# IML-DKFZ/values

Measured on AMD Instinct MI355X. Metric: uncertainty-volumes/sec (64^3, T=10 MC-dropout), higher is better.
Workload: dtype f32; 1 GPU; C2: 64^3 1-channel volumes, UNet3D(initial_filter_size=8, 2 classes), T=10 MC-dropout passes + fused softmax/entropy/MI/variance/argmax reduction; dropout=hash bit generator, new seed every step, weights=torch default init, seed 123

## Files before the change

include/values_amd.h:

```cpp
#ifndef VALUES_AMD_H
#define VALUES_AMD_H

#include <stddef.h>
#include <stdint.h>

#ifdef __cplusplus
extern "C" {
#endif

typedef void* vx_stream_t;

enum {
  VX_OK = 0,
  VX_E_NULL = -1,
  VX_E_SHAPE = -2,
  VX_E_DTYPE = -3,
  VX_E_WORKSPACE = -4,
  VX_E_ALIGN = -5
};

enum { VX_F32 = 0, VX_F64 = 1 };
enum { VX_ACT_NONE = 0, VX_ACT_LRELU = 1 , VX_ACT_RELU = 2 };
enum { VX_DROP_NONE = 0, VX_DROP_HASH = 1, VX_DROP_MASK = 2 };

// ... 107 lines not shown
  const float* acc_in;
  int32_t acc_pitch;
  int32_t out_planar, in_planar;
  int32_t products;
} vx_conv3d_args;
int64_t vx_conv3d_upfused_packed_floats(void);
int vx_pack_conv3d_upfused(const float* w1_torch, const float* b1, const float* up_w_torch, const float* up_b, float* packed,
                           vx_stream_t stream);
int vx_conv3d_k3_prologue_ok(int D, int H, int W, int Cin, int Cout);
int vx_conv3d_k3_upfuse_ok(int D, int H, int W, int Cin, int Cout);
int64_t vx_convT_zc16_packed_floats(void);
int64_t vx_conv3d_upfused_zc16_packed_floats(void);
int vx_pack_conv3d_upfused_zc16(const float* w1_torch, const float* up_w_torch, const float* up_b, float* packed, vx_stream_t stream);
int vx_pack_convT_zc16(const float* w_torch , float* packed, vx_stream_t stream);
int vx_conv3d_k3_skip_prologue_ok(int D, int H, int W, int Cin, int Cout, int xblk);
int vx_conv3d_k3_acc_ok(int D, int H, int W, int Cin, int Cout);
int vx_conv3d_k3_planar_ok(int D, int H, int W, int Cin, int Cout);
int vx_conv3d_k3_poolfuse_ok(int D, int H, int W, int Cin, int Cout);
int vx_conv3d_k3_presplit_ok(int D, int H, int W, int Cin, int Cout);
int vx_conv3d_k3_poolfin_ok(int Cin, int Cout);
int vx_prenorm_split(float* x, const float* mean, const float* rstd, int N, int64_t nvox, float scale, vx_stream_t stream);
int vx_pool_finish(const float* pool_raw, const uint32_t* pool_flags, const float* mean, const float* rstd, float* out,
                   int out_pitch, int N, int64_t voxels_per_sample, int drop_scale2, vx_stream_t stream);
int vx_pool_finish_z(const float* pool_raw, const uint32_t* pool_flags, const float* mean, const float* rstd, float* out,
                     int out_pitch, int N, int Dp, int64_t plane_voxels, int drop_scale2, vx_stream_t stream);
int vx_conv3d_k3_pool_layout(int D, int H, int W, int Cin, int Cout);
int vx_conv3d_k3_tiles(int D, int H, int W);
int vx_conv3d_k3_tiles_for(int D, int H, int W, int Cout);
int vx_conv3d_k3(const vx_conv3d_args* a, vx_stream_t stream);
int vx_conv3d_k3_head_fusable(int Cin, int Cout);
int vx_conv3d_k3_route(const vx_conv3d_args* a, char* kernel_name, int cap);

int vx_conv3d_k3_c1_tiles(int D, int H, int W);
int vx_conv3d_k3_c1(const float* in, const float* w_torch , const float* bias, float* out,
                    int out_pitch, int N, int D, int H, int W, int Cout, int repeat, const int32_t* src,
                    const int32_t* flip, float* stats_partial, vx_stream_t stream);

int vx_pack_input_cl8(const float* in, float* out, int N, int Cin, int D, int H, int W, int repeat, const int32_t* src,
                      const int32_t* flip, vx_stream_t stream);

int vx_instnorm_finalize(const float* stats_partial, int N, int ntiles, int C, int64_t nvox, float eps,
                         float* mean, float* rstd, vx_stream_t stream);

typedef struct vx_norm_args {
  const float* x; int32_t x_pitch;
  const float* mean; const float* rstd;
  float* out; int32_t out_pitch, out_coff;
  float* pool_out; int32_t pool_pitch;
  int32_t N, D, H, W, C;
  int32_t act, drop_mode; uint32_t drop_seed, drop_layer; const uint8_t* drop_mask;
  int32_t out_xblk, out_half;
  int32_t x_xblk, x_half;
  const uint32_t* seed_dev;
  uint32_t* range_flag;
} vx_norm_args;
int vx_norm_act_drop_pool(const vx_norm_args* a, vx_stream_t stream);
typedef struct vx_stat_src {
  const float* stats_partial; int32_t tiles; float eps; int64_t count;
  float* mean_out; float* rstd_out;
} vx_stat_src;
int vx_norm_act_drop_pool_stats(const vx_norm_args* a, const vx_stat_src* st, vx_stream_t stream);
int vx_prenorm_split_stats(float* x, const vx_stat_src* st, int N, int64_t nvox, float scale, vx_stream_t stream);
int vx_zero(void* p, int64_t bytes, vx_stream_t stream);
int vx_pool_finish_z_stats(const float* pool_raw, const uint32_t* pool_flags, const vx_stat_src* st, float* out, int out_pitch,
                           int N, int Dp, int64_t plane_voxels, int drop_scale2, vx_stream_t stream);
int vx_norm_act_drop_pool_bcast(const vx_norm_args* a, int x_repeat, vx_stream_t stream);
typedef struct vx_norm_route_info {
  int32_t grid_x, grid_y;
  uint32_t per_sample;
  uint32_t magic_pw, magic_c4, magic_rh;
} vx_norm_route_info;
int vx_norm_act_drop_pool_route(const vx_norm_args* a, int x_repeat, const vx_stat_src* st, char* kernel_name, int cap,
                                vx_norm_route_info* info);

typedef struct vx_convT_args {
  const float* in; int32_t in_pitch;
  const float* w_packed; const float* bias;
  float* out; int32_t out_pitch, out_coff;
  int32_t N, D, H, W, Cin, Cout;
  int32_t act, drop_mode; uint32_t drop_seed, drop_layer; const uint8_t* drop_mask;
  int32_t out_xblk, out_half;
  uint32_t* range_flag;
  const uint32_t* seed_dev;
} vx_convT_args;
int vx_convT_k2s2(const vx_convT_args* a, vx_stream_t stream);
typedef struct vx_convT_route_info {
  int32_t grid_x, grid_y;
} vx_convT_route_info;
int vx_convT_k2s2_route(const vx_convT_args* a, char* kernel_name, int cap, vx_convT_route_info* info);

int vx_conv1x1_ncdhw(const float* in, int in_pitch, const float* w, const float* bias, float* out, int N, int D,
                     int H, int W, int F, int C, const int32_t* dst, const int32_t* flip, vx_stream_t stream);

typedef struct vx_unet3d_weights {
  const float* conv_w[18];
  const float* conv_b[18];
  const float* up_w[4];
  const float* up_b[4];
  const float* final_w;
  const float* final_b;
  int32_t F;
  int32_t num_classes;
  int32_t conv_family[18];
  int32_t in_channels;
  int32_t no_instancenorm;
  const float* up_fused;
  const float* split_w[2];
  int32_t split_family;
  const float* up3_zc16;
  const float* up3_fused;
} vx_unet3d_weights;

typedef struct vx_unet3d_run {
  const float* x;
  int32_t N, D, H, W;
  int32_t repeat;
  const int32_t* src;
  const int32_t* flip;
  const int32_t* dst;
  int32_t drop_mode;
  uint32_t seed;
  const uint8_t* masks[17];
  float* logits;
  void* workspace; size_t workspace_bytes;
  uint32_t* range_flag;
  const uint32_t* seed_dev;
} vx_unet3d_run;

size_t vx_unet3d_workspace_bytes(int N, int D, int H, int W, int F);
int vx_unet3d_forward(const vx_unet3d_weights* w, const vx_unet3d_run* r, vx_stream_t stream);
int vx_unet3d_forward_profiled(const vx_unet3d_weights* w, const vx_unet3d_run* r, vx_stream_t stream,
                               int max_launches, float* ms, const char** labels, int* n_launches);

typedef struct vx_conv2d_args {
  const float* in; int32_t in_pitch;
  const float* w_packed; const float* bias;
  float* out; int32_t out_pitch, out_coff;
  int32_t N, H, W, Cin, Cout, KS, S;
  float* stats_partial;
  int32_t w_family;
  const float* in_scale; const float* in_shift;
  int32_t in_cpitch, in_group_images, in_relu;
  const float* out_scale; const float* out_shift;
  const float* out_add; int32_t out_add_pitch;
  int32_t out_act;
} vx_conv2d_args;
int64_t vx_conv2d_packed_floats(int Cin, int Cout, int KS);
int vx_pack_conv2d(const float* w_torch , float* w_packed, int Cin, int Cout, int KS, vx_stream_t stream);
int vx_conv2d_tiles(int H, int W, int KS, int S);
int vx_conv2d(const vx_conv2d_args* a, vx_stream_t stream);
typedef struct vx_conv2d_route_info {
  int32_t nchunks;
  int32_t w_all;
  int32_t lds_bytes;
  int32_t grid_x, grid_y;
} vx_conv2d_route_info;
int vx_conv2d_route(const vx_conv2d_args* a, char* kernel_name, int cap, vx_conv2d_route_info* info);

int vx_bn_finalize(const float* stats_partial, int ntiles, int C, int64_t count, float eps, const float* gamma,
                   const float* beta, float* scale, float* shift, vx_stream_t stream);
int vx_bn_finalize_groups(const float* stats_partial, int ntiles_per_group, int G, int C, int cpitch, int64_t count_per_group,
                          float eps, const float* gamma, const float* beta, float* scale, float* shift, vx_stream_t stream);

typedef struct vx_bn_affine_item {
  const float* gamma; const float* beta; const float* running_mean; const float* running_var;
  float* scale; float* shift;
  int32_t C, cpitch;
} vx_bn_affine_item;
int vx_bn_running_affine(const vx_bn_affine_item* items, int n_items, float eps, vx_stream_t stream);

typedef struct vx_affine_args {
  const float* x; int32_t x_pitch;
  const float* scale; const float* shift;
  const float* add; int32_t add_pitch;
  float* out; int32_t out_pitch, out_coff;
  int32_t N, H, W, C, OH, OW;
  int32_t act;
  int32_t drop_mode; uint32_t drop_seed, drop_layer; const uint8_t* drop_mask;
  int32_t group_images;
} vx_affine_args;
int vx_affine_gather(const vx_affine_args* a, vx_stream_t stream);

typedef struct vx_fuse_term {
  const float* x; int32_t x_pitch, H, W;
  const float* scale; const float* shift;
} vx_fuse_term;
typedef struct vx_fuse_args {
  vx_fuse_term term[4]; int32_t nterms;
  float* out; int32_t out_pitch;
  int32_t N, OH, OW, C;
  int32_t act;
  int32_t group_images;
} vx_fuse_args;
// ... 412 lines not shown
```

values_amd/_lib.py:

```python
from __future__ import annotations

import ctypes as C
import os

_HERE = os.path.dirname(os.path.abspath(__file__))
LIB_PATH = os.environ.get("VX_LIB_PATH") or os.path.join(_HERE, "libvalues_amd.so")

VX_F32, VX_F64 = 0, 1
VX_ACT_NONE, VX_ACT_LRELU, VX_ACT_RELU = 0, 1, 2
VX_DROP_NONE, VX_DROP_HASH, VX_DROP_MASK = 0, 1, 2

_p = C.c_void_p
_i = C.c_int
_i32 = C.c_int32
_u32 = C.c_uint32
_i64 = C.c_int64


class ConvArgs(C.Structure):
    _fields_ = [("in_", _p), ("w_packed", _p), ("bias", _p), ("out", _p),
                ("in_pitch", _i32), ("out_pitch", _i32), ("out_coff", _i32),
                ("N", _i32), ("D", _i32), ("H", _i32), ("W", _i32), ("Cin", _i32), ("Cout", _i32),
                ("act", _i32), ("drop_mode", _i32), ("drop_seed", _u32), ("drop_layer", _u32),
                ("drop_mask", _p), ("stats_partial", _p), ("in_xblk", _i32), ("w_family", _i32),
                ("head_out", _p), ("head_w", _p), ("head_b", _p), ("head_dst", _p), ("head_flip", _p),
                ("head_C", _i32),
                ("in_mean", _p), ("in_rstd", _p), ("in_drop_mode", _i32), ("in_drop_seed", _u32), ("in_drop_layer", _u32),
                ("in_repeat", _i32), ("out_xblk", _i32), ("out_half", _i32), ("range_flag", _p), ("seed_dev", _p),
                ("up_in", _p), ("up_w", _p), ("up_b", _p), ("up_pitch", _i32), ("pool_out", _p), ("pool_flags", _p),
                ("in_split", _i32), ("out_f16", _i32), ("in_f16", _i32),
                ("out_split", _i32), ("up_split", _i32), ("up_fused", _p), ("in_pool_flags", _p),
                ("acc_in", _p), ("acc_pitch", _i32), ("out_planar", _i32), ("in_planar", _i32), ("products", _i32)]


class NormArgs(C.Structure):
    _fields_ = [("x", _p), ("x_pitch", _i32), ("mean", _p), ("rstd", _p),
                ("out", _p), ("out_pitch", _i32), ("out_coff", _i32),
                ("pool_out", _p), ("pool_pitch", _i32),
                ("N", _i32), ("D", _i32), ("H", _i32), ("W", _i32), ("C", _i32),
                ("act", _i32), ("drop_mode", _i32), ("drop_seed", _u32), ("drop_layer", _u32), ("drop_mask", _p),
                ("out_xblk", _i32), ("out_half", _i32), ("x_xblk", _i32), ("x_half", _i32), ("seed_dev", _p),
                ("range_flag", _p)]


class StatSrc(C.Structure):
    _fields_ = [("stats_partial", _p), ("tiles", _i32), ("eps", C.c_float), ("count", _i64), ("mean_out", _p), ("rstd_out", _p)]


class NormRouteInfo(C.Structure):
    _fields_ = [("grid_x", _i32), ("grid_y", _i32), ("per_sample", _u32), ("magic_pw", _u32), ("magic_c4", _u32), ("magic_rh", _u32)]


class ConvTArgs(C.Structure):
    _fields_ = [("in_", _p), ("in_pitch", _i32), ("w_packed", _p), ("bias", _p),
                ("out", _p), ("out_pitch", _i32), ("out_coff", _i32),
                ("N", _i32), ("D", _i32), ("H", _i32), ("W", _i32), ("Cin", _i32), ("Cout", _i32),
                ("act", _i32), ("drop_mode", _i32), ("drop_seed", _u32), ("drop_layer", _u32), ("drop_mask", _p),
                ("out_xblk", _i32), ("out_half", _i32), ("range_flag", _p), ("seed_dev", _p)]


class ConvTRouteInfo(C.Structure):
    _fields_ = [("grid_x", _i32), ("grid_y", _i32)]


class Conv2dArgs(C.Structure):
    _fields_ = [("in_", _p), ("in_pitch", _i32), ("w_packed", _p), ("bias", _p),
                ("out", _p), ("out_pitch", _i32), ("out_coff", _i32),
                ("N", _i32), ("H", _i32), ("W", _i32), ("Cin", _i32), ("Cout", _i32), ("KS", _i32), ("S", _i32),
                ("stats_partial", _p), ("w_family", _i32),
                ("in_scale", _p), ("in_shift", _p), ("in_cpitch", _i32), ("in_group_images", _i32), ("in_relu", _i32),
                ("out_scale", _p), ("out_shift", _p), ("out_add", _p), ("out_add_pitch", _i32), ("out_act", _i32)]


class Conv2dRouteInfo(C.Structure):
    _fields_ = [("nchunks", _i32), ("w_all", _i32), ("lds_bytes", _i32), ("grid_x", _i32), ("grid_y", _i32)]


class BnAffineItem(C.Structure):
    _fields_ = [("gamma", _p), ("beta", _p), ("running_mean", _p), ("running_var", _p), ("scale", _p), ("shift", _p),
                ("C", _i32), ("cpitch", _i32)]


class AffineArgs(C.Structure):
    _fields_ = [("x", _p), ("x_pitch", _i32), ("scale", _p), ("shift", _p), ("add", _p), ("add_pitch", _i32),
                ("out", _p), ("out_pitch", _i32), ("out_coff", _i32),
                ("N", _i32), ("H", _i32), ("W", _i32), ("C", _i32), ("OH", _i32), ("OW", _i32),
                ("act", _i32), ("drop_mode", _i32), ("drop_seed", _u32), ("drop_layer", _u32), ("drop_mask", _p),
                ("group_images", _i32)]


class FuseTerm(C.Structure):
    _fields_ = [("x", _p), ("x_pitch", _i32), ("H", _i32), ("W", _i32), ("scale", _p), ("shift", _p)]


class FuseArgs(C.Structure):
    _fields_ = [("term", FuseTerm * 4), ("nterms", _i32), ("out", _p), ("out_pitch", _i32),
                ("N", _i32), ("OH", _i32), ("OW", _i32), ("C", _i32), ("act", _i32), ("group_images", _i32)]


class Config(C.Structure):
    _fields_ = [(n, _i32) for n in (
        "conv_fp32", "s16_no_prenorm", "s16_no_xp8", "s16_skip_raw", "no_head_fusion", "s16_no_upfuse", "s16_no_poolfuse",
        "storage16", "s16_generic", "s16_no_zc16", "s16_no_halves", "s16_no_deep", "s16_no_l1dma", "c2s_no_wide", "c2s_no_oct")]
    RETIRED = ("s16_no_upcompose", "s16_no_upsplit", "s16_no_poolfin", "s16_no_presplit", "s16_no_dbplain")


def _retired_field(name):
    def put(self, v):
        if v:
            raise ValueError(f"vx_config.{name} was retired in 0.7.0: the default data flow is the only one")
    return property(lambda self: 0, put)


for _n in Config.RETIRED:
    setattr(Config, _n, _retired_field(_n))


class UncOutputs(C.Structure):
    _fields_ = [("mean_prob", _p), ("pred_entropy", _p), ("exp_entropy", _p), ("mutual_info", _p), ("variance", _p),
                ("argmax", _p), ("sample_argmax", _p), ("in_count", _p), ("out_count", _p)]


class UNet3DWeights(C.Structure):
    _fields_ = [("conv_w", _p * 18), ("conv_b", _p * 18), ("up_w", _p * 4), ("up_b", _p * 4),
                ("final_w", _p), ("final_b", _p), ("F", _i32), ("num_classes", _i32), ("conv_family", _i32 * 18),
                ("in_channels", _i32), ("no_instancenorm", _i32), ("up_fused", _p), ("split_w", _p * 2), ("split_family", _i32), ("up3_zc16", _p), ("up3_fused", _p)]


class UNet3DRun(C.Structure):
    _fields_ = [("x", _p), ("N", _i32), ("D", _i32), ("H", _i32), ("W", _i32), ("repeat", _i32),
                ("src", _p), ("flip", _p), ("dst", _p), ("drop_mode", _i32), ("seed", _u32),
                ("masks", _p * 17), ("logits", _p), ("workspace", _p), ("workspace_bytes", C.c_size_t),
                ("range_flag", _p), ("seed_dev", _p)]


VX_NIFTI_COPY, VX_NIFTI_PROB, VX_NIFTI_MEAN_PROB, VX_NIFTI_ARGMAX, VX_NIFTI_ARGMAX_MEAN = 0, 1, 2, 3, 4


class NiftiItem(C.Structure):
    _fields_ = [("src", _p), ("count", _p), ("dst_off", _i64), ("kind", _i32), ("src_dtype", _i32), ("esize", _i32),
                ("T", _i32), ("C", _i32), ("t", _i32), ("c", _i32), ("X", _i32), ("Y", _i32), ("Z", _i32),
                ("header", C.c_uint8 * 352)]


class GzItem(C.Structure):
    _fields_ = [("src", _p), ("n", _i64), ("dst_off", _i64), ("stride_hint", _i32 * 3), ("pad", _i32)]


class PngItem(C.Structure):
    _fields_ = [("labels", _p), ("ignore", _p), ("H", _i32), ("W", _i32)]


class PngRgbItem(C.Structure):
    _fields_ = [("rgb", _p), ("H", _i32), ("W", _i32)]


class InflateItem(C.Structure):
    _fields_ = [("src", _p), ("src_n", _i64), ("dst_off", _i64), ("dst_cap", _i64), ("format", _i32), ("pad", _i32)]


VX_INFLATE_GZIP, VX_INFLATE_ZLIB, VX_INFLATE_RAW = 0, 1, 2
INFLATE_STATUS = ("ok", "truncated", "bad header", "bad block type", "invalid code lengths", "bad symbol",
                  "distance beyond the output start", "output capacity reached", "checksum mismatch", "ISIZE mismatch",
                  "trailing bytes", "stored block length mismatch", "preset dictionary")
VX_INFLATE_CAPACITY = 7


class NiftiDecItem(C.Structure):
    _fields_ = [("src", _p), ("src_n", _i64), ("vox_offset", _i64), ("dst", _p), ("dst_n", _i64), ("ndim", _i32),
                ("dims", _i32 * 7), ("code", _i32), ("big_endian", _i32), ("out_dtype", _i32), ("pad", _i32),
                ("slope", C.c_double), ("inter", C.c_double)]


class PngUnfilterItem(C.Structure):
    _fields_ = [("src", _p), ("src_n", _i64), ("dst", _p), ("H", _i32), ("W", _i32), ("bpp", _i32), ("pad", _i32)]


VX_PNG_OK, VX_PNG_BAD_FILTER, VX_PNG_BAD_SIZE = 0, 1, 2
PNG_STATUS = ("ok", "filter byte above 4", "stream size is not H (1 + W bpp)")


class TiffLzwItem(C.Structure):
    _fields_ = [("src", _p), ("src_n", _i64), ("dst_off", _i64), ("dst_cap", _i64)]


class TiffUnpredictItem(C.Structure):
    _fields_ = [("src", _p), ("dst", _p), ("rows", _i32), ("W", _i32), ("predictor", _i32), ("pad", _i32)]


VX_LZW_OK, VX_LZW_TRUNCATED, VX_LZW_BAD_CODE = 0, 1, 2
LZW_STATUS = ("ok", "truncated", "bad code")
VX_LZW_NO_ROOM = 3


VX_AGG_IMAGE, VX_AGG_THRESHOLD, VX_AGG_PATCH = 0, 1, 2
VX_AGG_MAX_SPECS, VX_AGG_MAX_ITEMS = 8, 4096


class AggItem(C.Structure):
    _fields_ = [("map", _p), ("dtype", _i32), ("D", _i32), ("H", _i32), ("W", _i32)]


class AggSpec(C.Structure):
    _fields_ = [("kind", _i32), ("pd", _i32), ("ph", _i32), ("pw", _i32), ("thr", C.c_double)]


VX_EM_MAX_ITEMS = 4096


# ... 62 lines not shown


class Gather3dItem(C.Structure):
    _fields_ = [("src", _p), ("kind", _i32), ("dims", _i32 * 3), ("origin", _i32 * 3), ("reserved", _i32)]


class Acc3dItem(C.Structure):
    _fields_ = [("sum", _p), ("count", _p), ("dims", _i32 * 3), ("origin", _i32 * 3)]


class CompositeLabel(C.Structure):
    _fields_ = [("ptr", _p), ("kind", _i32), ("flags", _i32)]


class CompositeItem(C.Structure):
    _fields_ = [("image", _p), ("count", _p), ("data", _p), ("gt_seg", _p), ("gt", _p), ("image_kind", _i32),
                ("first_label", _i32), ("R", _i32), ("dims", _i32 * 3)]


VX_MSR_MAX_ITEMS, VX_MSR_MAX_PLANES = 65536, 1 << 22


class MsrItem(C.Structure):
    _fields_ = [("out", _p), ("n", _i64), ("first_plane", _i32), ("C", _i32), ("dtype", _i32), ("reserved", _i32)]


SIGNATURES = {
    "vx_version": (_i, []),
    "vx_last_error_string": (C.c_char_p, []),
    "vx_last_kernel_name": (C.c_char_p, []),
    "vx_drop_hash_mask": (_i, [_u32, _u32, _i, _i64, _p, _p]),
    "vx_get_config": (_i, [C.POINTER(Config)]),
    "vx_set_config": (_i, [C.POINTER(Config)]),
    "vx_conv3d_k3_family": (_i, [_i, _i]),
    "vx_conv2d_family": (_i, [_i, _i, _i]),
    "vx_unc_reduce": (_i, [_p, _i, _i, _i, _i, _i, _i64, _p, _p, _p, _p, _p, _p, _p]),
    "vx_unc_reduce_ex": (_i, [_p, _i, _i, _i, _i, _i, _i64, C.POINTER(UncOutputs), _p]),
    "vx_unc_stats_accumulate": (_i, [_p, _i, _i, _i, _i64, _p, _p]),
    "vx_unc_stats_finalize": (_i, [_p, _i, _i, _i, _i64, _p, _p, _p, _p, _p, _p]),
    "vx_softmax_planar": (_i, [_p, _i64, _i, _i64, _p, _p]),
    "vx_one_minus_msr": (_i, [_p, _i, _i, _i64, _p, _p]),
    "vx_one_minus_msr_batched_workspace_bytes": (_i64, [_i, _i]),
    "vx_one_minus_msr_batched": (_i, [C.POINTER(MsrItem), _i, C.POINTER(_p), _i, _p, _i64, _p]),
    "vx_conv3d_k3_packed_floats": (_i64, [_i, _i]),
    "vx_pack_conv3d_k3": (_i, [_p, _p, _i, _i, _p]),
    "vx_convT_k2s2_packed_floats": (_i64, [_i, _i]),
    "vx_pack_convT_k2s2": (_i, [_p, _p, _i, _i, _p]),
    "vx_conv3d_k3_tiles": (_i, [_i, _i, _i]),
    "vx_conv3d_k3_tiles_for": (_i, [_i, _i, _i, _i]),
    "vx_conv3d_k3_head_fusable": (_i, [_i, _i]),
    "vx_conv3d_k3_route": (_i, [C.POINTER(ConvArgs), C.c_char_p, _i]),
    "vx_conv3d_k3_prologue_ok": (_i, [_i, _i, _i, _i, _i]),
    "vx_conv3d_k3_upfuse_ok": (_i, [_i, _i, _i, _i, _i]),
    "vx_conv3d_k3_poolfuse_ok": (_i, [_i, _i, _i, _i, _i]),
    "vx_conv3d_k3_presplit_ok": (_i, [_i, _i, _i, _i, _i]),
    "vx_conv3d_k3_poolfin_ok": (_i, [_i, _i]),
    "vx_conv3d_upfused_packed_floats": (_i64, []),
    "vx_pack_conv3d_upfused": (_i, [_p, _p, _p, _p, _p, _p]),
    "vx_pack_conv3d_upfused_zc16": (_i, [_p, _p, _p, _p, _p]),
    "vx_conv3d_upfused_zc16_packed_floats": (_i64, []),
    "vx_pool_finish": (_i, [_p, _p, _p, _p, _p, _i, _i, _i64, _i, _p]),
    "vx_pool_finish_z": (_i, [_p, _p, _p, _p, _p, _i, _i, _i, _i64, _i, _p]),
    "vx_conv3d_k3_pool_layout": (_i, [_i, _i, _i, _i, _i]),
    "vx_conv3d_k3_skip_prologue_ok": (_i, [_i, _i, _i, _i, _i, _i]),
    "vx_conv3d_k3_acc_ok": (_i, [_i, _i, _i, _i, _i]),
    "vx_conv3d_k3_planar_ok": (_i, [_i, _i, _i, _i, _i]),
    "vx_convT_zc16_packed_floats": (_i64, []),
    "vx_pack_convT_zc16": (_i, [_p, _p, _p]),
    "vx_prenorm_split": (_i, [_p, _p, _p, _i, _i64, C.c_float, _p]),
    "vx_zero": (_i, [_p, _i64, _p]),
    "vx_conv3d_k3": (_i, [C.POINTER(ConvArgs), _p]),
    "vx_conv3d_k3_c1_tiles": (_i, [_i, _i, _i]),
    "vx_conv3d_k3_c1": (_i, [_p, _p, _p, _p, _i, _i, _i, _i, _i, _i, _i, _p, _p, _p, _p]),
    "vx_pack_input_cl8": (_i, [_p, _p, _i, _i, _i, _i, _i, _i, _p, _p, _p]),
    "vx_instnorm_finalize": (_i, [_p, _i, _i, _i, _i64, C.c_float, _p, _p, _p]),
    "vx_norm_act_drop_pool": (_i, [C.POINTER(NormArgs), _p]),
    "vx_norm_act_drop_pool_bcast": (_i, [C.POINTER(NormArgs), _i, _p]),
    "vx_norm_act_drop_pool_stats": (_i, [C.POINTER(NormArgs), C.POINTER(StatSrc), _p]),
    "vx_norm_act_drop_pool_route": (_i, [C.POINTER(NormArgs), _i, C.POINTER(StatSrc), C.c_char_p, _i, C.POINTER(NormRouteInfo)]),
    "vx_prenorm_split_stats": (_i, [_p, C.POINTER(StatSrc), _i, _i64, C.c_float, _p]),
    "vx_pool_finish_z_stats": (_i, [_p, _p, C.POINTER(StatSrc), _p, _i, _i, _i, _i64, _i, _p]),
    "vx_convT_k2s2": (_i, [C.POINTER(ConvTArgs), _p]),
    "vx_convT_k2s2_route": (_i, [C.POINTER(ConvTArgs), C.c_char_p, _i, C.POINTER(ConvTRouteInfo)]),
    "vx_conv1x1_ncdhw": (_i, [_p, _i, _p, _p, _p, _i, _i, _i, _i, _i, _i, _p, _p, _p]),
    "vx_unet3d_workspace_bytes": (C.c_size_t, [_i, _i, _i, _i, _i]),
    "vx_unet3d_forward": (_i, [C.POINTER(UNet3DWeights), C.POINTER(UNet3DRun), _p]),
    "vx_unet3d_forward_profiled": (_i, [C.POINTER(UNet3DWeights), C.POINTER(UNet3DRun), _p, _i, C.POINTER(C.c_float),
                                        C.POINTER(C.c_char_p), C.POINTER(_i)]),
    "vx_softmax_accumulate": (_i, [_p, _i, _i, _i, _i, _i, _i, _p, _p, _p, _i, _i, _i, _i, _p]),
    "vx_aleatoric_sample": (_i, [_p, _p, _u32, _i, _i, _i, _i64, _p, _p, _p]),
    "vx_colorize_u8": (_i, [_p, _p, _i64, _p, _i, _p, _p]),
    "vx_fuse_sum": (_i, [C.POINTER(FuseArgs), _p]),
    "vx_tta_views_2d": (_i, [_p, _i, _p, _p, C.POINTER(C.c_float), C.POINTER(C.c_float), C.c_float, _i, _i, _i, _i,
                             C.POINTER(C.c_int32), _p, _p]),
    "vx_tta_views_2d_gen": (_i, [_p, _i, _p, _p, C.POINTER(C.c_float), C.POINTER(C.c_float), C.c_float, _i, _i, _i, _i,
                                 C.POINTER(C.c_int32), _u32, _p, _i64, C.POINTER(C.c_float), _p, _p, _p]),
    "vx_noise_view_3d": (_i, [_p, _p, _i, _i64, _u32, _p, _i64, C.c_float, C.c_float, _i, _p, _p]),
    "vx_count_nonzero_batched_workspace_bytes": (_i64, [_i]),
    "vx_count_nonzero_batched": (_i, [C.POINTER(CountItem), _i, _p, _p, _i64, _p]),
    "vx_select_segments_workspace_bytes": (_i64, [_i]),
    "vx_select_segments": (_i, [C.POINTER(SelectItem), _i, _i64, _p, _p, _p, _i64, _p]),
    "vx_volume_stats_batched_workspace_bytes": (_i64, [C.POINTER(PrepItem), _i]),
    "vx_volume_stats_batched": (_i, [C.POINTER(PrepItem), _i, _p, _p, _i64, _p]),
    "vx_zscore_pad_batched_workspace_bytes": (_i64, [C.POINTER(PrepPadItem), _i]),
    "vx_zscore_pad_batched": (_i, [C.POINTER(PrepPadItem), _i, _p, _p, _i64, _p]),
    "vx_p2d_out_size": (_i, [_i, _i]),
    "vx_crop_resize_batched_workspace_bytes": (_i64, [C.POINTER(P2dItem), _i, C.POINTER(P2dTables)]),
    "vx_crop_resize_batched": (_i, [C.POINTER(P2dItem), _i, C.POINTER(P2dTables), _p, _p, _i64, _p]),
    "vx_label_switch_batched_workspace_bytes": (_i64, [_i, _i]),
    "vx_label_switch_batched": (_i, [C.POINTER(LswitchItem), _i, _i, C.POINTER(LswitchRow), _i, _p, _u32, C.POINTER(C.c_float), _p,
                                     _p, _i64, _p]),
    "vx_gather_patches_3d_workspace_bytes": (_i64, [_i]),
    "vx_gather_patches_3d": (_i, [C.POINTER(Gather3dItem), _i, _p, _i, _i, _i, _p, _i64, _p]),
    "vx_softmax_accumulate_cases_workspace_bytes": (_i64, [_i]),
    "vx_softmax_accumulate_cases": (_i, [_p, _i, _i, _i, _i, _i, _i, C.POINTER(Acc3dItem), _i, _p, _i64, _p]),
    "vx_case_composite_workspace_bytes": (_i64, [_i, _i]),
    "vx_case_composite": (_i, [C.POINTER(CompositeItem), _i, C.POINTER(CompositeLabel), _i, _p, _p, _i64, _p]),
    "vx_toy_embed": (_i, [_p, C.POINTER(_i32), C.POINTER(_i32), C.c_double, _i, _i, _p, C.POINTER(_i32), _p]),
    "vx_gauss_blur_axis_f64": (_i, [_p, _p, C.POINTER(_i32), _i, _p, _i, _p]),
    "vx_count_ge_f64": (_i, [_p, _i64, C.c_double, _p, _p]),
    "vx_order_stats_f64_workspace_bytes": (_i64, [_i]),
    "vx_order_stats_f64_reads": (_i, [_i64, C.POINTER(_i64), _i]),
    "vx_order_stats_f64": (_i, [_p, _i64, C.POINTER(_i64), _i, _p, _p, _p, _i64, _p]),
    "vx_toy_segment": (_i, [_p, _i64, C.POINTER(C.c_double), _i, _p, _p]),
    "vx_toy_noise": (_i, [_p, _i64, _u32, _u32, C.c_double, _p]),
    "vx_voxelize_meshes": (_i, [_p, C.POINTER(_i64), _i, C.POINTER(C.c_double), C.c_double, C.POINTER(_i32), _p, _p, _p]),
    "vx_mask_agreement": (_i, [_p, _i, _i, _i64, _p, _p]),
    "vx_mask_agreement_batched": (_i, [_p, _i, _i, _i, _i64, _i, _p, _p]),
    "vx_soft_metric_workspace_bytes": (_i64, [_i, _i]),
    "vx_soft_metric_sums": (_i, [_p, _p, _i, _i, _i64, _p, _p, _p]),
    "vx_soft_metric_batched_workspace_bytes": (_i64, [_i, _i, _i, _i64]),
    "vx_soft_metric_sums_batched": (_i, [_p, _p, _i, _i, _i, _i64, _p, _p, _p]),
    "vx_val_sums_workspace_bytes": (_i64, [_i, _i, _i64]),
    "vx_val_sums_batched": (_i, [_p, _p, _i, _i, _i64, _i, _p, _p, _i64, _p]),
    "vx_val_aleatoric_sums_workspace_bytes": (_i64, [_i, _i, _i64]),
    "vx_val_aleatoric_sums_batched": (_i, [_p, _p, _u32, _u32, _p, _i, _i, _i, _i64, _i, _p, _p, _i64, _p]),
    "vx_val_ssn_sums_workspace_bytes": (_i64, [_i, _i, _i, _i64]),
    "vx_val_ssn_sums_batched": (_i, [_p, _p, _p, _u32, _u32, _p, _i, _i, _i, _i, _i64, C.c_float, _i, _p, _p, _p, _i64, _p]),
    "vx_ssn2d_lowres": (_i, [_p, _i, _p, _i, _p, _u32, _i, _i64, _i, _i, _i, _p, _p, _p]),
    "vx_ssn2d_add_diag": (_i, [_p, _p, _p, _u32, _i, _i, _i64, C.c_float, _p]),
    "vx_softmax_variance": (_i, [_p, _i, _i, _i, _i, _i64, _p, _p]),
    "vx_ssn_sample": (_i, [_p, _p, _p, _u32, _i, _i, _i, _i, _i64, C.c_float, _p, _p]),
    "vx_conv2d_packed_floats": (_i64, [_i, _i, _i]),
    "vx_pack_conv2d": (_i, [_p, _p, _i, _i, _i, _p]),
    "vx_conv2d_tiles": (_i, [_i, _i, _i, _i]),
    "vx_conv2d": (_i, [C.POINTER(Conv2dArgs), _p]),
    "vx_conv2d_route": (_i, [C.POINTER(Conv2dArgs), C.c_char_p, _i, C.POINTER(Conv2dRouteInfo)]),
    "vx_bn_finalize": (_i, [_p, _i, _i, _i64, C.c_float, _p, _p, _p, _p, _p]),
    "vx_bn_finalize_groups": (_i, [_p, _i, _i, _i, _i, _i64, C.c_float, _p, _p, _p, _p, _p]),
    "vx_bn_running_affine": (_i, [_p, _i, C.c_float, _p]),
    "vx_affine_gather": (_i, [C.POINTER(AffineArgs), _p]),
    "vx_bilinear_nchw": (_i, [_p, _i, _i, _i, _i, _i, _i, _i, _p, _p, _p, _p]),
    "vx_bilinear_softmax_nchw": (_i, [_p, _i, _i, _i, _i, _i, _i, _i, _p, _p, _p, _p]),
    "vx_ncc_batched_workspace_bytes": (C.c_size_t, [C.POINTER(NccItem), _i]),
    "vx_ncc_batched": (_i, [C.POINTER(NccItem), _i, _p, _p, C.c_size_t, _p]),
    "vx_rater_variance": (_i, [_p, _i, _i64, _p, _p]),
    "vx_platt_batched_workspace_bytes": (C.c_size_t, [C.POINTER(EmItem), _i]),
    "vx_platt_sums_batched": (_i, [C.POINTER(EmItem), _i, C.POINTER(C.c_double), _i, _p, _p, C.c_size_t, _p]),
    "vx_calib_batched_workspace_bytes": (C.c_size_t, [C.POINTER(EmItem), _i]),
    "vx_calib_bins_batched": (_i, [C.POINTER(EmItem), _i, C.POINTER(C.c_double), C.POINTER(C.c_double), _i, _p, _p,
                                   C.c_size_t, _p]),
    "vx_aggregate_workspace_bytes": (C.c_size_t, [C.POINTER(AggItem), _i, C.POINTER(AggSpec), _i]),
    "vx_aggregate_batched": (_i, [C.POINTER(AggItem), _i, C.POINTER(AggSpec), _i, _p, _p, C.c_size_t, _p]),
    "vx_nifti_workspace_bytes": (C.c_size_t, [_i]),
    "vx_nifti_payload_bytes": (_i64, [C.POINTER(NiftiItem)]),
    "vx_nifti_payload": (_i, [C.POINTER(NiftiItem), _i, _p, _i64, _p, C.c_size_t, _p]),
# ... 137 lines not shown
```

values_amd/csrc/conv3d_deep.hip:

```cpp
#include "s16_common.h"
#include "conv3d_internal.h"

struct DeepArgs {
  vx_conv3d_args a;
  const float* w;
  int tx, ty, tz, ts;
  int ltx, lty, ltz;
  int tiles_x, tiles_y, tiles_z;
  int npos;
  int nchunks, ncg;
  unsigned m_cg, m_tx, m_ty, m_tz;
  int stat_epc;
  int stat_parts;
  int nfull, tail0, tail_wgs, ltail;
  unsigned long long* stamps;
  int abl;
};

#define DP_STAMP VX_STAMP
#define DP_WAIT_LOADS VX_STAMP_WAIT_LOADS
#define DP_ABL VX_DIAG(ka.abl)

constexpr int DEEP_PREC_B = DEEP_NPOS * 16;
constexpr int DEEP_IMG_B = 2 * DEEP_PREC_B;
// ... 240 lines not shown
      ly = v & (TY - 1); v >>= ka.lty;
      lz = v & (TZ - 1); smp = v >> ka.ltz;
    };
#pragma unroll
    for (int r = 0; r < R; ++r) {
      int cx_, ly, lz, smp;
      vox_of((wave * R + r) * 16 + m, cx_, ly, lz, smp);
      vbase[r] = (((smp * HZ + lz) * HY + ly) * HX + cx_) * 16;
    }
    int toff[NSTEP];
#pragma unroll
    for (int s = 0; s < NSTEP; ++s) {
      int tap = 4 * s + g;
      if (DP_ABL & 64) tap = 4 * s;
      if (tap > 26) tap = 26;
      toff[s] = (((tap / 9) * HY + (tap / 3) % 3) * HX + tap % 3) * 16;
    }
    const unsigned char* wlane = s_w + lane * 16;
    const bool f_lrelu = EPI == 3 ? a.act == VX_ACT_LRELU : EPI == 1;
    const bool f_relu = EPI == 3 && a.act == VX_ACT_RELU;
    const uint32_t seed_out = EPI == 1 ? vx_seed_of(a, a.drop_seed) : 0u;

    f32x4 acc[R][NT], accx[R][NT];

    auto multiply = [&](int buf) {
      const unsigned char* img = s_img + buf * DEEP_IMG_B;
      const unsigned char* wb = wlane + buf * DEEP_W_B;
      f16x8 wh[NT], wl[NT], bh[2][R], bl[R];
      int vb_[R];
#pragma unroll
      for (int r = 0; r < R; ++r) { vb_[r] = vbase[r]; asm volatile("" : "+v"(vb_[r])); }
      auto ldA = [&](int s, int nt) {
        wh[nt] = *reinterpret_cast<const f16x8*>(wb + ((s * NT + nt) * 2) * 1024);
        wl[nt] = *reinterpret_cast<const f16x8*>(wb + ((s * NT + nt) * 2 + 1) * 1024);
      };
      auto ldBh = [&](int s, int r) { bh[s & 1][r] = *reinterpret_cast<const f16x8*>(img + vb_[r] + toff[s]); };
      auto ldBl = [&](int s, int r) { bl[r] = *reinterpret_cast<const f16x8*>(img + vb_[r] + toff[s] + DEEP_PREC_B); };
#pragma unroll
      for (int nt = 0; nt < NT; ++nt) ldA(0, nt);
#pragma unroll
      for (int r = 0; r < R; ++r) { ldBh(0, r); ldBl(0, r); }
      __builtin_amdgcn_sched_group_barrier(0x100, 2 * NT + 2 * R, 0);
#pragma unroll
      for (int s = 0; s < NSTEP; ++s) {
        const bool more = s + 1 < NSTEP;
        const int set = s & 1;
#pragma unroll
        for (int nt = 0; nt < NT; ++nt) {
#pragma unroll
          for (int r = 0; r < R; ++r) {
            acc[r][nt] = __builtin_amdgcn_mfma_f32_16x16x32_f16(wh[nt], bh[set][r], acc[r][nt], 0, 0, 0);
            accx[r][nt] = __builtin_amdgcn_mfma_f32_16x16x32_f16(wh[nt], bl[r], accx[r][nt], 0, 0, 0);
            if (more && nt == 0) ldBh(s + 1, r);
            if (more && nt == NT - 1) ldBl(s + 1, r);
          }
#pragma unroll
          for (int r = 0; r < R; ++r) accx[r][nt] = __builtin_amdgcn_mfma_f32_16x16x32_f16(wl[nt], bh[set][r], accx[r][nt], 0, 0, 0);
          if (more) ldA(s + 1, nt);
        }
#ifndef DEEP_NO_PIPE
#pragma unroll
        for (int nt = 0; nt < NT; ++nt) {
#pragma unroll
          for (int r = 0; r < R; ++r) {
            __builtin_amdgcn_sched_group_barrier(0x008, 2, 0);
            if (more) __builtin_amdgcn_sched_group_barrier(0x100, 1, 0);
          }
          __builtin_amdgcn_sched_group_barrier(0x008, R, 0);
          if (more) __builtin_amdgcn_sched_group_barrier(0x100, 2, 0);
        }
#endif
      }
    };

    auto epilogue = [&](int ci) {
      float* red = s_red + (ci & 1) * (NW * 32 * 2);
      int n0, tzi, tyi, txi, cg;
      pair_of(ci, n0, tzi, tyi, txi, cg);
      const auto kp = kernarg();
      const unsigned vox0 = (unsigned)(((tzi * TZ) * a.H + tyi * TY) * a.W + txi * TX);
      const unsigned osoff = (vox0 * (unsigned)out_voxf + (unsigned)(cg * 32)) * 4u;
      const __amdgpu_buffer_rsrc_t osrd = __builtin_amdgcn_make_buffer_rsrc(
          (void*)(reinterpret_cast<char*>(kp->a.out) + (size_t)n0 * out_sample * 4), 0, VX_NUMREC, 0x00020000);
      float ssum[NT][4], ssq[NT][4];
      if (STATS) {
#pragma unroll
        for (int nt = 0; nt < NT; ++nt)
#pragma unroll
          for (int j = 0; j < 4; ++j) { ssum[nt][j] = 0.f; ssq[nt][j] = 0.f; }
      }
      int m_ = m;
      asm volatile("" : "+v"(m_));
#pragma unroll
      for (int r = 0; r < R; ++r) {
        int cx_, ly, lz, smp;
        vox_of((wave * R + r) * 16 + m_, cx_, ly, lz, smp);
        const int ovox = (lz * a.H + ly) * a.W + cx_;
        unsigned ovoff_r = ((unsigned)smp * (unsigned)out_sample + (unsigned)ovox * (unsigned)out_voxf + (unsigned)kp->a.out_coff + 4u * g) * 4u;
        if constexpr (R == 2) {
          if (n0 + smp >= a.N) ovoff_r = VX_OOB;
        }
        uint32_t hword = 0;
        if (EPI == 1) {
          const vx_dkey key = vx_drop_key(seed_out, kp->a.drop_layer, (uint32_t)(n0 + smp));
          hword = vx_drop_word(key, (vox0 + (unsigned)ovox) * (unsigned)ka.ncg + (unsigned)cg) >> (4 * g);
        }
#pragma unroll
        for (int nt = 0; nt < NT; ++nt) {
          f32x4 v;
#pragma unroll
          for (int j = 0; j < 4; ++j) v[j] = fmaf(accx[r][nt][j], 1.0f / 2048.f, acc[r][nt][j]);
          if (STATS) {
#pragma unroll
            for (int j = 0; j < 4; ++j) { ssum[nt][j] += v[j]; ssq[nt][j] = fmaf(v[j], v[j], ssq[nt][j]); }
          }
          if (f_lrelu) {
#pragma unroll
            for (int j = 0; j < 4; ++j) v[j] = fmaxf(v[j], 0.01f * v[j]);
          } else if (f_relu) {
#pragma unroll
            for (int j = 0; j < 4; ++j) v[j] = fmaxf(v[j], 0.f);
          }
          if (EPI == 1) {
            const uint32_t bits = hword >> (16 * nt);
#pragma unroll
            for (int j = 0; j < 4; ++j) v[j] *= __uint_as_float((bits << (30 - j)) & 0x40000000u);
          }
          if (!STATS) rmax = vx_max3abs(vx_max3abs(rmax, v[0], v[1]), v[2], v[3]);
          u32x4 sv = __builtin_bit_cast(u32x4, v);
          if (EPI == 1 || EPI == 3) {
            if (a.out_split) {
              typedef unsigned u32x2 __attribute__((ext_vector_type(2)));
              f16x4 hi, lo;
              vx_split4_s(v, hi, lo);
              const u32x2 h2 = __builtin_bit_cast(u32x2, hi), l2 = __builtin_bit_cast(u32x2, lo);
              sv = (u32x4){h2[0], h2[1], l2[0], l2[1]};
            }
          }
          __builtin_amdgcn_raw_buffer_store_b128(sv, osrd, (int)ovoff_r, (int)(osoff + (unsigned)(nt * 64)), 0);
          __builtin_amdgcn_sched_barrier(0);
          asm volatile("s_nop 3" ::: "memory");
          __builtin_amdgcn_sched_barrier(0);
        }
      }
      if (STATS) {
#pragma unroll
        for (int nt = 0; nt < NT; ++nt)
#pragma unroll
          for (int j = 0; j < 4; ++j) {
            float s = ssum[nt][j], qq = ssq[nt][j];
#pragma unroll
            for (int rot = 8; rot >= 1; rot >>= 1) { s += vx_row_ror(s, rot); qq += vx_row_ror(qq, rot); }
            if (m == 0) {
              red[(wave * 32 + nt * 16 + g * 4 + j) * 2 + 0] = s;
              red[(wave * 32 + nt * 16 + g * 4 + j) * 2 + 1] = qq;
            }
          }
      }
    };

    auto flush_tile = [&](int ci) {
      const float* red = s_red + (ci & 1) * (NW * 32 * 2);
      int n0, tzi, tyi, txi, cg;
      pair_of(ci, n0, tzi, tyi, txi, cg);
      const auto kp = kernarg();
      const int epc = kp->stat_epc;
      const int tps = ka.tiles_x * ka.tiles_y * ka.tiles_z;
      const int tile = (tzi * ka.tiles_y + tyi) * ka.tiles_x + txi;
      float* dst = kp->a.stats_partial + (((size_t)n0 * tps + tile) * epc * a.Cout + cg * 32) * 2;
      const int parts = kp->stat_parts, wpp = NW / parts;
      const int ltail = kp->ltail;
      const bool shared = ci >= nfull && ltail > 0;
      const int p = tid >> 5, ch = tid & 31;
      if (p < parts && (!shared || (p * wpp) >> (3 - ltail) == (vb & ((1 << ltail) - 1)))) {
        float s = 0.f, qq = 0.f;
#pragma unroll
        for (int i = 0; i < NW; ++i) {
          const int w = (p * wpp + i) & (NW - 1);
          const float rs = red[(w * 32 + ch) * 2 + 0], rq = red[(w * 32 + ch) * 2 + 1];
          s = i < wpp ? s + rs : s;
          qq = i < wpp ? qq + rq : qq;
        }
        dst[(size_t)p * a.Cout * 2 + ch * 2 + 0] = s;
        dst[(size_t)p * a.Cout * 2 + ch * 2 + 1] = qq;
      }
      if (!shared || (vb & ((1 << ltail) - 1)) == 0)
        for (int e = parts; e < epc; ++e)
          if (tid < 64) dst[(size_t)e * a.Cout * 2 + tid] = 0.f;
    };

    const bool late = wave >= NW / 2;
    const bool tail_mine = (wave >> (3 - ka.ltail)) == (vb & ((1 << ka.ltail) - 1));
    Cur cx = {0, 0};
    int j = 0;
    int prev_ci = -1;
    int fl_ci = -1, fl_at = 0;
    while (cx.ci < npair_wg) {
      __syncthreads();
      DP_STAMP(0);
      if (STATS && fl_ci >= 0 && j >= fl_at && !late) { flush_tile(fl_ci); fl_ci = -1; }
      if (late && prev_ci >= 0) {
        if (!(DP_ABL & 2)) epilogue(prev_ci);
        prev_ci = -1;
      }
      DP_STAMP(2);
      const bool mine = cx.ci < nfull || tail_mine;
      if (cx.c == 0 && mine) {
        int n0, tzi, tyi, txi, cg;
        pair_of(cx.ci, n0, tzi, tyi, txi, cg);
        const f32x4 zero = {0.f, 0.f, 0.f, 0.f};
#pragma unroll
        for (int nt = 0; nt < NT; ++nt) {
          const f32x4 b4 = *reinterpret_cast<const f32x4*>(s_bias + cg * 32 + nt * 16 + 4 * g);
#pragma unroll
          for (int r = 0; r < R; ++r) { acc[r][nt] = b4; accx[r][nt] = zero; }
        }
      }
      if (mine && !(DP_ABL & 1)) multiply(j & 1);
      DP_STAMP(1);
      if (cx.c == NCH - 1) {
        if (mine) {
          if (late) prev_ci = cx.ci;
          else if (!(DP_ABL & 2)) epilogue(cx.ci);
        }
        if (STATS) { fl_ci = cx.ci; fl_at = j + 2; }
      }
      DP_STAMP(2);
#ifdef VX_CONV_STAMPS
      ++st_iters;
#endif
      advance(cx);
      ++j;
    }
    if (late && prev_ci >= 0) epilogue(prev_ci);
    if (STATS) {
      __syncthreads();
      if (fl_ci >= 0 && !late) flush_tile(fl_ci);
    }
  }
  if (!STATS && a.range_flag) {
    float mx = rmax;
#pragma unroll
    for (int off = 32; off >= 1; off >>= 1) mx = fmaxf(mx, __shfl_xor(mx, off, 64));
    if (lane == 0 && !(mx < 32768.f)) atomicMax(a.range_flag, __float_as_uint(mx));
  }
#ifdef VX_CONV_STAMPS
  if (ka.stamps && lane == 0) {
    unsigned long long* d = ka.stamps + ((size_t)blockIdx.x * 16 + wave) * 8;
    for (int i = 0; i < 6; ++i) d[i] = st_sum[i];
    d[6] = st_iters;
  }
#endif
}

__global__ void pack_conv3d_deep_kernel(const float* __restrict__ w, _Float16* __restrict__ out, int Cin, int64_t total) {
  const int nch = Cin / 8;
  for (int64_t i = (int64_t)blockIdx.x * blockDim.x + threadIdx.x; i < total; i += (int64_t)gridDim.x * blockDim.x) {
    const int j = (int)(i & 7), lane = (int)((i >> 3) & 63), hl = (int)((i >> 9) & 1), nt = (int)((i >> 10) & 1);
    const int64_t sb = i >> 11;
    const int step = (int)(sb % 7);
    const int64_t blk = sb / 7;
    const int chunk = (int)(blk % nch), cg = (int)(blk / nch);
    const int row = cg * 32 + nt * 16 + (lane & 15), tap = 4 * step + (lane >> 4);
    const float v = tap > 26 ? 0.f : w[((size_t)row * Cin + 8 * chunk + j) * 27 + tap];
    const float c = fminf(fmaxf(v, -65504.f), 65504.f);
    const _Float16 h = (_Float16)c;
    out[i] = hl == 0 ? h : (_Float16)((v - (float)h) * 2048.f);
  }
}

int vx_pack_conv3d_deep(const float* w_torch, float* w_packed, int Cin, int Cout, hipStream_t s) {
  const int64_t total = conv3d_deep_packed_floats(Cin, Cout) * 2;
  if (total <= 0) return VX_OK;
  int blocks = (int)((total + 255) / 256);
  if (blocks > 4096) blocks = 4096;
  hipLaunchKernelGGL(pack_conv3d_deep_kernel, dim3(blocks), dim3(256), 0, s, w_torch, reinterpret_cast<_Float16*>(w_packed), Cin, total);
  VX_CHECK_LAUNCH("vx_pack_conv3d_k3(deep)");
  return VX_OK;
}

template <int R, int EPI, int PRE>
static int launch_deep(const DeepArgs& ka, const Conv3dRoute& r, int grid, hipStream_t s) {
  constexpr size_t lds = 2 * (size_t)DEEP_IMG_B + 2 * (size_t)DEEP_W_B + 2 * 8 * 32 * 2 * 4 + DEEP_MAXC * 4;
  static_assert(lds <= 160 * 1024, "LDS budget");
  auto kern = conv3d_deep_kernel<R, EPI, PRE>;
  static bool attr = false;
  if (!attr) {
    hipError_t e = hipFuncSetAttribute(reinterpret_cast<const void*>(kern), hipFuncAttributeMaxDynamicSharedMemorySize, (int)lds);
    if (e != hipSuccess) VX_FAIL((int)e, "vx_conv3d_k3(deep): hipFuncSetAttribute(%zu B LDS): %s", lds, hipGetErrorString(e));
    attr = true;
  }
  static const char* kname = vx_conv3d_kname(r);
  vx_note_kernel(kname);
  hipLaunchKernelGGL(kern, dim3((unsigned)grid), dim3(768), lds, s, ka);
  VX_CHECK_LAUNCH("vx_conv3d_k3(deep)");
  return VX_OK;
// ... 26 lines not shown
```

values_amd/csrc/conv3d_k3.hip:

```cpp
#include <string.h>

#include "conv3d_internal.h"

extern "C" int vx_conv3d_k3_route(const vx_conv3d_args* ap, char* kernel_name, int cap) {
  if (!ap) VX_FAIL(VX_E_NULL, "vx_conv3d_k3: null args");
  Conv3dRoute r;
  const int rc = conv3d_route(*ap, vx_cfg(), &r);
  if (rc != VX_OK) VX_FAIL(rc, "%s", r.err);
  if (kernel_name && cap > 0) conv3d_route_name(r, kernel_name, cap);
  return VX_OK;
}

extern "C" int vx_conv3d_k3(const vx_conv3d_args* ap, vx_stream_t stream) {
  if (!ap) VX_FAIL(VX_E_NULL, "vx_conv3d_k3: null args");
  const vx_conv3d_args& a = *ap;
  Conv3dRoute r;
  const int rc = conv3d_route(a, vx_cfg(), &r);
  if (rc != VX_OK) VX_FAIL(rc, "%s", r.err);
  hipStream_t s = (hipStream_t)stream;
  switch (r.kernel) {
    case CONV3D_C8: return vx_conv3d_c8_launch(r, a, s);
    case CONV3D_XP8W: return vx_conv3d_xp8w_launch(r, a, s);
    case CONV3D_ZC16: return vx_conv3d_zc16_launch(r, a, a.w_packed + r.w_off, s);
    case CONV3D_DEEP: return vx_conv3d_deep_launch(r, a, a.w_packed + r.w_off, s);
    case CONV3D_S16: return vx_conv3d_s16_launch(r, a, s);
    default: return vx_conv3d_mfma_launch(r, a, s);
  }
}

extern "C" int vx_conv3d_k3_family(int Cin, int Cout) { return conv3d_family(Cin, Cout, vx_cfg()); }
extern "C" int64_t vx_conv3d_k3_packed_floats(int Cin, int Cout) { return conv3d_packed_floats(Cin, Cout, vx_cfg()); }

extern "C" int vx_pack_conv3d_k3(const float* w_torch, float* w_packed, int Cin, int Cout, vx_stream_t stream) {
  if (!w_torch || !w_packed) VX_FAIL(VX_E_NULL, "vx_pack_conv3d_k3: null pointer");
  const int64_t total = vx_conv3d_k3_packed_floats(Cin, Cout);
  if (total < 0) VX_FAIL(VX_E_SHAPE, "vx_pack_conv3d_k3: Cin=%d Cout=%d must be positive multiples of 8", Cin, Cout);
  const ConvCfg c = conv_config(Cin, Cout, vx_cfg());
  hipStream_t s = (hipStream_t)stream;
  if (c.C8) return vx_pack_conv3d_k3_c8(w_torch, w_packed, Cin, s);
  if (!c.S16) return vx_pack_conv3d_k3_mfma(w_torch, w_packed, Cin, Cout, total, s);
  const int rc = vx_pack_conv3d_k3_s16(w_torch, w_packed, Cin, Cout, s);
  if (rc != VX_OK) return rc;
  float* w_block = w_packed + conv3d_s16_packed_floats(Cin, Cout);
  if (conv3d_deep_packs(Cin, Cout)) return vx_pack_conv3d_deep(w_torch, w_block, Cin, Cout, s);
  return vx_pack_conv3d_zc16(w_torch, w_block, Cin, Cout, s);
}

extern "C" int vx_conv3d_k3_tiles(int D, int H, int W) { return conv3d_tiles_max(D, H, W); }
extern "C" int vx_conv3d_k3_tiles_for(int D, int H, int W, int Cout) { return conv3d_tiles_for(D, H, W, Cout, vx_cfg()); }
extern "C" int vx_conv3d_k3_head_fusable(int Cin, int Cout) { return conv3d_head_fusable(Cin, Cout, vx_cfg()); }
extern "C" int vx_conv3d_k3_prologue_ok(int D, int H, int W, int Cin, int Cout) { return conv3d_prologue_ok(D, H, W, Cin, Cout, vx_cfg()); }
extern "C" int vx_conv3d_k3_skip_prologue_ok(int D, int H, int W, int Cin, int Cout, int xblk) {
  return conv3d_skip_prologue_ok(D, H, W, Cin, Cout, xblk, vx_cfg());
}
extern "C" int vx_conv3d_k3_acc_ok(int D, int H, int W, int Cin, int Cout) { return conv3d_zc16_16to16(D, H, W, Cin, Cout, vx_cfg()) ? 1 : 0; }
extern "C" int vx_conv3d_k3_planar_ok(int D, int H, int W, int Cin, int Cout) { return conv3d_zc16_16to16(D, H, W, Cin, Cout, vx_cfg()) ? 1 : 0; }
extern "C" int vx_conv3d_k3_upfuse_ok(int D, int H, int W, int Cin, int Cout) { return conv3d_upfuse_ok(D, H, W, Cin, Cout, vx_cfg()); }
extern "C" int vx_conv3d_k3_pool_layout(int D, int H, int W, int Cin, int Cout) { return conv3d_pool_layout(D, H, W, Cin, Cout, vx_cfg()); }
extern "C" int vx_conv3d_k3_poolfuse_ok(int D, int H, int W, int Cin, int Cout) { return conv3d_pool_layout(D, H, W, Cin, Cout, vx_cfg()) != 0 ? 1 : 0; }
extern "C" int vx_conv3d_k3_presplit_ok(int D, int H, int W, int Cin, int Cout) { return conv3d_presplit_ok(D, H, W, Cin, Cout, vx_cfg()); }
extern "C" int vx_conv3d_k3_poolfin_ok(int Cin, int Cout) { return conv3d_poolfin_ok(Cin, Cout, vx_cfg()); }
```

values_amd/csrc/conv3d_route.h:

```cpp
#pragma once
#include <stdint.h>
#include <stdio.h>

#include "../../include/values_amd.h"
#include "host_checks.h"

constexpr int DEEP_NPOS = 1080;
constexpr int DEEP_NPOS_R2 = 896;
constexpr int DEEP_W_B = 7 * 2 * 2 * 1024;
constexpr int DEEP_MAXC = 512;
constexpr int DEEP_MAXDIM = 32;
constexpr int S16_HEAD_MAXC = 4;

enum Conv3dKernel { CONV3D_MFMA = 0, CONV3D_C8, CONV3D_S16, CONV3D_XP8W, CONV3D_ZC16, CONV3D_DEEP, CONV3D_NKERNELS };

#define MFMA_TILES(X, CB, NT, XP) X(CB, NT, 16, 4, 4, 8, XP) X(CB, NT, 8, 8, 4, 8, XP) X(CB, NT, 4, 4, 4, 4, XP)
#define MFMA_INSTANCES(X) MFMA_TILES(X, 8, 1, 1) MFMA_TILES(X, 16, 1, 0) MFMA_TILES(X, 16, 2, 0) MFMA_TILES(X, 8, 1, 0) MFMA_TILES(X, 8, 2, 0)
#define C8_INSTANCES(X) X(1, 32, 4, 4) X(2, 32, 4, 4) X(1, 16, 8, 4) X(2, 16, 8, 4) X(1, 8, 4, 4) X(2, 8, 4, 4)
#define S16_SMALL(X, CB, NT, XP)                                                                                       \
  X(CB, NT, 16, 4, 4, 8, XP, 0, 0) X(CB, NT, 16, 4, 4, 8, XP, 0, 1) X(CB, NT, 16, 4, 4, 8, XP, 0, 3)                     \
  X(CB, NT, 8, 8, 4, 8, XP, 0, 0) X(CB, NT, 8, 8, 4, 8, XP, 0, 1) X(CB, NT, 8, 8, 4, 8, XP, 0, 3) X(CB, NT, 4, 4, 4, 4, XP, 0, 3)
#define S16_LARGE(X, CB, XP) X(CB, 1, 16, 8, 4, 8, XP, 0, 0) X(CB, 1, 16, 8, 4, 8, XP, 0, 1) X(CB, 1, 16, 8, 4, 8, XP, 0, 3)
#define S16_DB_PLAIN(X, CB, NT) X(CB, NT, 16, 4, 4, 8, 0, 2, 0) X(CB, NT, 16, 4, 4, 8, 0, 2, 1) X(CB, NT, 16, 4, 4, 8, 0, 2, 3)
#define S16_DB_XP(X)                                                                                                   \
// ... 306 lines not shown
               "statistics epilogue (contr_1_2)");
  int epi;
  if (a.stats_partial) epi = a.pool_out ? 4 : 0;
  else if (a.head_out) epi = 2;
  else if (a.drop_mode == VX_DROP_HASH) epi = 1;
  else epi = 3;
  if (epi == 2 && a.act == VX_ACT_LRELU && a.drop_mode == VX_DROP_NONE) epi = 5;
  if (epi == 2 && !(a.act == VX_ACT_LRELU && a.drop_mode == VX_DROP_HASH)) return ROUTE_DECLINED;
  if (epi == 1 && a.act != VX_ACT_LRELU) return ROUTE_DECLINED;
  const int up = a.up_in ? (a.up_fused ? 2 : 1) : 0;
  if (a.pool_out && nch != 1) VX_REFUSE(r, VX_E_SHAPE, "vx_conv3d_k3(xp8w): the pooled output goes with Cin = 8");
  if (a.out_split) VX_REFUSE(r, VX_E_SHAPE, "vx_conv3d_k3(xp8w): out_split is an epilogue of the tile kernel");
  if (a.up_split && !up) VX_REFUSE(r, VX_E_SHAPE, "vx_conv3d_k3(xp8w): up_split without up_in");
  if (a.out_f16 && (epi != 1 || a.out_xblk || a.out_coff))
    VX_REFUSE(r, VX_E_SHAPE, "vx_conv3d_k3(xp8w): fp16 output goes with the LeakyReLU + dropout epilogue and a dense output tensor");
  if (a.in_f16 && !(nch == 1 && epi == 2 && pre == 0 && !up && !a.in_xblk))
    VX_REFUSE(r, VX_E_SHAPE, "vx_conv3d_k3(xp8w): fp16 input goes with the dense 8-channel layer that carries the fused head");
  const int in16 = (a.in_f16 ? 1 : 0) | (a.products == 1 ? 2 : 0);
  route_instance(r, CONV3D_XP8W, 6, nch, epi, pre, up, nch == 2 ? 8 : 4, in16);
  if (conv3d_instance_exists(CONV3D_XP8W, r->p, 6)) return VX_OK;
  if (a.products == 1 && !a.in_f16)
    VX_REFUSE(r, VX_E_SHAPE, "vx_conv3d_k3(xp8w): products = 1 exists for the MC-dropout forward's contr_1_2, upscale2 + expand_1_1 and "
               "expand_1_2 + head (nch %d, epilogue %d, prologue %d, up %d)", nch, epi, pre, up);
  if (up) VX_REFUSE(r, VX_E_SHAPE, "vx_conv3d_k3(xp8w): no fused up-convolution for this epilogue (act=%d, drop_mode=%d, statistics=%d)",
                     a.act, a.drop_mode, a.stats_partial ? 1 : 0);
  if (a.pool_out) VX_REFUSE(r, VX_E_SHAPE, "vx_conv3d_k3(xp8w): no pooled output for this epilogue");
  return ROUTE_DECLINED;
}

static inline int route_zc16(const vx_conv3d_args& a, int stat_tiles, Conv3dRoute* r) {
  if (a.in_xblk || a.head_out || a.in_split || a.in_f16 || a.out_f16 || (a.in_repeat > 1)) return ROUTE_DECLINED;
  if ((a.in_planar || a.out_planar) && (a.drop_mode == VX_DROP_MASK || !a.out || a.in_pitch != a.Cin || a.Cout != 16))
    VX_REFUSE(r, VX_E_SHAPE, "vx_conv3d_k3(zc16): the planar pre-split hand-over needs hash or no dropout and dense 16-channel tensors");
  if (a.up_in && (a.Cin != 16 || a.in_mean || a.stats_partial || a.up_pitch < 32 || a.up_pitch % 4 || (a.up_fused && (!a.acc_in || a.out_xblk || a.out_split))))
    VX_REFUSE(r, VX_E_SHAPE, "vx_conv3d_k3(zc16): the fused up-convolution (32 coarse channels -> the conv's 16 input channels) goes with an "
               "activation epilogue, no prologue, up_pitch >= 32 (got %d), up_w packed by vx_pack_convT_zc16; composed weights "
               "(up_fused: vx_pack_conv3d_upfused_zc16) only together with partial sums (acc_in) and a dense float or planar output", a.up_pitch);
  if (a.drop_mode == VX_DROP_MASK || !a.out) return ROUTE_DECLINED;
  route_columns(r, a, 2, stat_tiles);
  const int cps = r->tiles_x * r->tiles_y;
  if ((int64_t)a.N * cps >= (1ll << 31)) VX_REFUSE(r, VX_E_SHAPE, "vx_conv3d_k3(zc16): too many columns");
  if (a.in_pitch != a.Cin) return ROUTE_DECLINED;
  if (a.stats_partial && (stat_tiles % cps || a.act != VX_ACT_NONE || (a.drop_mode != VX_DROP_NONE && !a.pool_out)))
    VX_REFUSE(r, VX_E_SHAPE, "vx_conv3d_k3(zc16): statistics go with a plain epilogue");
  if (a.pool_out && (!a.stats_partial || a.Cin != 16)) VX_REFUSE(r, VX_E_SHAPE, "vx_conv3d_k3(zc16): the pooled output goes with statistics, 16 -> 16");
  int pre = 0;
  if (a.in_pool_flags) pre = 3;
  else if (a.in_mean) pre = 1;
  if ((pre == 1 && a.Cin != 16) || (pre == 3 && a.Cin != 8)) return ROUTE_DECLINED;
  if (a.in_planar) {
    if (a.Cin != 16 || pre != 0 || a.up_in || a.acc_in || a.stats_partial || !vx_aligned16(a.in) ||
        (vx_wide)a.D * a.H * a.W * 64 >= CONV3D_2GIB)
      VX_REFUSE(r, VX_E_SHAPE, "vx_conv3d_k3(zc16): a planar pre-split input (in_planar) goes with 16 -> 16, an activation epilogue, no "
                 "prologue / up-convolution / partial sums, a 16-byte aligned tensor, one sample below 2 GiB");
    pre = 4;
  }
  if (a.out_planar && (a.stats_partial || a.out_pitch != 16 || a.out_coff != 0 || a.out_xblk || a.out_split || a.out == a.acc_in ||
                       (vx_wide)a.D * a.H * a.W * 64 >= CONV3D_2GIB))
    VX_REFUSE(r, VX_E_SHAPE, "vx_conv3d_k3(zc16): a planar pre-split output (out_planar) goes with an activation epilogue into a dense "
               "16-channel tensor that is not the partial sums' (another layout), one sample below 2 GiB");
  int epi;
  if (a.stats_partial) epi = a.pool_out ? 4 : 0;
  else if (a.drop_mode == VX_DROP_HASH) { if (a.act != VX_ACT_LRELU) return ROUTE_DECLINED; epi = 1; }
  else epi = 3;
  if (a.out_split && a.stats_partial) VX_REFUSE(r, VX_E_SHAPE, "vx_conv3d_k3(zc16): out_split goes with the activation epilogues");
  if (a.out_planar) {
    if (a.Cin != 16 || pre != 0 || (epi != 1 && epi != 3) || ((a.acc_in != nullptr) != (a.up_in != nullptr)))
      VX_REFUSE(r, VX_E_SHAPE, "vx_conv3d_k3(zc16): out_planar goes with 16 -> 16, an activation epilogue, no prologue, and either partial "
                 "sums + the fused up-convolution together or neither");
    epi = epi == 1 ? 5 : 6;
  }
  if (a.acc_in && (a.Cin != 16 || pre != 0 || a.stats_partial || a.acc_pitch < 16 || a.acc_pitch % 4 || !vx_aligned16(a.acc_in) ||
                   (vx_wide)a.D * a.H * a.W * a.acc_pitch * 4 >= CONV3D_2GIB))
    VX_REFUSE(r, VX_E_SHAPE, "vx_conv3d_k3(zc16): partial sums (acc_in) go with 16 -> 16, no prologue, an activation epilogue, a "
               "16-byte aligned tensor of pitch >= 16 (pitch %d), one sample below 2 GiB", a.acc_pitch);
  route_instance(r, CONV3D_ZC16, 5, a.Cin, epi, pre, a.acc_in ? 1 : 0, a.up_in ? 1 : 0);
  if (conv3d_instance_exists(CONV3D_ZC16, r->p, 5)) return VX_OK;
  if (a.up_in && !a.acc_in) VX_REFUSE(r, VX_E_SHAPE, "vx_conv3d_k3(zc16): no fused up-convolution for this epilogue");
  return ROUTE_DECLINED;
}

static inline int route_deep(const vx_conv3d_args& a, int stat_tiles, Conv3dRoute* r) {
  if (a.head_out || a.in_split || a.in_f16 || a.out_f16 || (a.in_repeat > 1) || a.out_xblk || a.up_in || a.pool_out ||
      a.in_pool_flags || a.acc_in)
    return ROUTE_DECLINED;
  if (a.drop_mode == VX_DROP_MASK || !a.out) return ROUTE_DECLINED;
  DeepGeo g;
  const int R = deep_pick(a.D, a.H, a.W, &g);
  if (!R) return ROUTE_DECLINED;
  if (a.in_xblk) {
    const int csrc = a.Cin / 2;
    if (a.in_mean || csrc % 8 || a.W % a.in_xblk) return ROUTE_DECLINED;
  } else if (a.in_pitch % 4) {
    return ROUTE_DECLINED;
  }
  if (a.in_mean && (a.in_pitch != a.Cin || g.ts != 1)) return ROUTE_DECLINED;
  if (a.stats_partial && g.ts != 1) return ROUTE_DECLINED;
  r->tx = g.tx; r->ty = g.ty; r->tz = g.tz; r->ts = g.ts; r->npos = g.npos;
  r->tiles_x = g.tiles_x; r->tiles_y = g.tiles_y; r->tiles_z = g.tiles_z;
  r->nchunks = a.Cin / 8;
  r->ncg = a.Cout / 32;
  const int tps = g.tiles_x * g.tiles_y * g.tiles_z;
  const int64_t npairs = (((int64_t)a.N + g.ts - 1) / g.ts) * tps * r->ncg;
  if (npairs >= (1ll << 31)) VX_REFUSE(r, VX_E_SHAPE, "vx_conv3d_k3(deep): too many tiles");
  r->nitems = (int)npairs;
  r->m_cg = vx_magic_raw(r->ncg); r->mx = vx_magic_raw(g.tiles_x); r->my = vx_magic_raw(g.tiles_y); r->mz = vx_magic_raw(g.tiles_z);
  r->stat_epc = 0;
  r->stat_parts = 1;
  r->tail_cap = 4;
  if (a.stats_partial) {
    if (stat_tiles % tps) return ROUTE_DECLINED;
    if (a.act != VX_ACT_NONE || a.drop_mode != VX_DROP_NONE) VX_REFUSE(r, VX_E_SHAPE, "vx_conv3d_k3(deep): statistics go with a plain epilogue");
    r->stat_epc = stat_tiles / tps;
    r->tail_cap = r->stat_parts = deep_stat_parts(r->stat_epc);
  }
  if ((vx_wide)g.ts * a.D * a.H * a.W * a.out_pitch * 4 >= CONV3D_2GIB)
    VX_REFUSE(r, VX_E_SHAPE, "vx_conv3d_k3(deep): one tile's samples must stay below 2 GiB");
  int epi;
  if (a.stats_partial) epi = 0;
  else if (a.drop_mode == VX_DROP_HASH) { if (a.act != VX_ACT_LRELU) return ROUTE_DECLINED; epi = 1; }
  else epi = 3;
  if (a.out_split && a.stats_partial) VX_REFUSE(r, VX_E_SHAPE, "vx_conv3d_k3(deep): out_split goes with the activation epilogues");
  route_instance(r, CONV3D_DEEP, 3, R, epi, a.in_mean ? 1 : 0);
  return conv3d_instance_exists(CONV3D_DEEP, r->p, 3) ? VX_OK : ROUTE_DECLINED;
}

static inline int route_s16(const vx_conv3d_args& a, const vx_config& cfg, Conv3dRoute* r) {
  const S16Cfg c = s16_config(a.Cin, a.Cout);
  int txv, ty, tz;
  vx_conv3d_s16_tile(a.H, a.W, a.Cout, &txv, &ty, &tz);
  const int tx = c.XP ? txv / 2 : txv;
  route_tiles(r, a, txv, ty, tz);
  r->nchunks = a.Cin / c.CB;
  r->ty8 = (tx == 16 && ty == 8) ? 1 : 0;
  const bool generic = cfg.s16_generic != 0;
  int epi = 3;
  if (generic) epi = 3;
  else if (a.act == VX_ACT_NONE && a.drop_mode == VX_DROP_NONE && !a.head_out && a.out) epi = 0;
  else if (a.act == VX_ACT_LRELU && a.drop_mode == VX_DROP_HASH && !a.head_out && a.out) epi = 1;
  else if (a.act == VX_ACT_LRELU && a.drop_mode == VX_DROP_HASH && a.head_out && c.XP) epi = 2;
  int db = 0;
  if (!generic && tx == 16 && c.XP && r->ty8 && r->nchunks <= 2) db = r->nchunks == 1 ? 2 : 3;
  if (!generic && tx == 16 && !c.XP && !r->ty8 && r->nchunks == 1) db = 2;
  if (epi == 2 && db != 2) epi = 3;
  if (db == 3 && epi == 0) epi = 3;
  if (tx == 4) epi = 3;
  route_instance(r, CONV3D_S16, 9, c.CB, c.NT, tx, ty, tz, tx == 4 ? 4 : 8, c.XP, db, epi);
  if (!conv3d_instance_exists(CONV3D_S16, r->p, 9)) VX_REFUSE(r, VX_E_SHAPE, "vx_conv3d_k3(s16): no instance for this tile");
  return VX_OK;
}

static inline int conv3d_route(const vx_conv3d_args& a, const vx_config& cfg, Conv3dRoute* r) {
  r->err[0] = 0;
  r->w_off = 0;
  if (!a.in || !a.w_packed || !a.bias || (!a.out && !a.head_out)) VX_REFUSE(r, VX_E_NULL, "vx_conv3d_k3: null tensor pointer");
  const ConvCfg c = conv_config(a.Cin, a.Cout, cfg);
  if (a.head_out) {
    if (!a.head_w || !a.head_b) VX_REFUSE(r, VX_E_NULL, "vx_conv3d_k3: fused head without weights");
    if (a.head_C < 1 || a.head_C > 8) VX_REFUSE(r, VX_E_SHAPE, "vx_conv3d_k3: fused head takes 1..8 classes, got %d", a.head_C);
    if (c.S16 && a.head_C > S16_HEAD_MAXC)
      VX_REFUSE(r, VX_E_SHAPE, "vx_conv3d_k3: the split-fp16 kernel fuses heads of up to 4 classes, got %d", a.head_C);
    if (!conv3d_head_fusable(a.Cin, a.Cout, cfg))
      VX_REFUSE(r, VX_E_SHAPE, "vx_conv3d_k3: no fused head for Cin=%d Cout=%d (see vx_conv3d_k3_head_fusable)", a.Cin, a.Cout);
    if (a.stats_partial) VX_REFUSE(r, VX_E_SHAPE, "vx_conv3d_k3: fused head on a layer with InstanceNorm statistics");
  }
  if (!conv3d_channels_ok(a.Cin, a.Cout))
    VX_REFUSE(r, VX_E_SHAPE, "vx_conv3d_k3: Cin=%d Cout=%d must be positive multiples of 8", a.Cin, a.Cout);
  if (a.N <= 0 || a.D <= 0 || a.H <= 0 || a.W <= 0) VX_REFUSE(r, VX_E_SHAPE, "vx_conv3d_k3: empty tensor");
  if (a.w_family != conv3d_family(a.Cin, a.Cout, cfg))
    VX_REFUSE(r, VX_E_DTYPE, "vx_conv3d_k3: weights packed for kernel family %d, the library is configured for family %d "
               "(vx_conv3d_k3_family(%d, %d)): re-pack them", a.w_family, conv3d_family(a.Cin, a.Cout, cfg), a.Cin, a.Cout);
  if (a.out_xblk && ((a.out_xblk != 1 && a.out_xblk != 2 && a.out_xblk != 4) || a.W % a.out_xblk || (a.out_half != 0 && a.out_half != 1)))
    VX_REFUSE(r, VX_E_SHAPE, "vx_conv3d_k3: bad concat output (xblk=%d, half=%d, W=%d)", a.out_xblk, a.out_half, a.W);
  if ((a.in_mean == nullptr) != (a.in_rstd == nullptr)) VX_REFUSE(r, VX_E_NULL, "vx_conv3d_k3: in_mean / in_rstd must come together");
  if (a.products != 0 && a.products != 1 && a.products != 3)
    VX_REFUSE(r, VX_E_SHAPE, "vx_conv3d_k3: products = %d (0 / 3: the default split scheme, 1: one fp16 product)", a.products);
  const bool xp8 = c.S16 && conv3d_xp8_applies(a.D, a.H, a.W, a.Cin, a.Cout, cfg) && a.drop_mode != VX_DROP_MASK;
  if (a.products == 1 && !(xp8 && a.in_drop_mode != VX_DROP_MASK))
    VX_REFUSE(r, VX_E_SHAPE, "vx_conv3d_k3: products = 1 is taken by the full-resolution z-column kernel only (got %dx%dx%d, %d -> %d)",
               a.D, a.H, a.W, a.Cin, a.Cout);
  if ((a.in_planar || a.out_planar) && !conv3d_zc16_16to16(a.D, a.H, a.W, a.Cin, a.Cout, cfg))
    VX_REFUSE(r, VX_E_SHAPE, "vx_conv3d_k3: the planar pre-split hand-over (in_planar / out_planar) is taken where vx_conv3d_k3_planar_ok "
               "(got %dx%dx%d, %d -> %d)", a.D, a.H, a.W, a.Cin, a.Cout);
  if (a.up_in) {
    if (!a.up_w || !a.up_b) VX_REFUSE(r, VX_E_NULL, "vx_conv3d_k3: fused up-convolution without weights");
    if (!conv3d_upfuse_ok(a.D, a.H, a.W, a.Cin, a.Cout, cfg) || a.drop_mode == VX_DROP_MASK || a.stats_partial || a.head_out)
      VX_REFUSE(r, VX_E_SHAPE, "vx_conv3d_k3: no fused up-convolution for this layer (see vx_conv3d_k3_upfuse_ok; hash or no "
                 "dropout, no statistics, no head): %dx%dx%d, %d -> %d", a.D, a.H, a.W, a.Cin, a.Cout);
    if (a.up_pitch < 16 || a.up_pitch % 4 || !vx_aligned16(a.up_in) || !vx_aligned16(a.up_b))
      VX_REFUSE(r, VX_E_ALIGN, "vx_conv3d_k3: up_in pitch %d (>= 16, multiple of 4 floats) / alignment", a.up_pitch);
    if ((vx_wide)(a.D / 2 + 2) * (a.H / 2) * (a.W / 2) * a.up_pitch * 4 >= CONV3D_2GIB)
      VX_REFUSE(r, VX_E_SHAPE, "vx_conv3d_k3: one coarse sample must stay below 2 GiB");
    if (a.up_fused && !vx_aligned16(a.up_fused)) VX_REFUSE(r, VX_E_ALIGN, "vx_conv3d_k3: up_fused alignment");
  } else if (a.up_fused) {
    VX_REFUSE(r, VX_E_SHAPE, "vx_conv3d_k3: up_fused (composed up-convolution weights) without up_in");
  }
  if (a.pool_out) {
    if (!a.pool_flags || !a.stats_partial) VX_REFUSE(r, VX_E_NULL, "vx_conv3d_k3: pool_out goes with pool_flags and stats_partial");
    if (!conv3d_pool_layout(a.D, a.H, a.W, a.Cin, a.Cout, cfg) || a.drop_mode == VX_DROP_MASK || a.act != VX_ACT_NONE || a.head_out)
      VX_REFUSE(r, VX_E_SHAPE, "vx_conv3d_k3: no pooled output for this layer (see vx_conv3d_k3_poolfuse_ok; hash or no dropout, "
                 "no activation): %dx%dx%d, %d -> %d", a.D, a.H, a.W, a.Cin, a.Cout);
    if (!vx_aligned16(a.pool_out)) VX_REFUSE(r, VX_E_ALIGN, "vx_conv3d_k3: pool_out alignment");
  }
  if (a.in_drop_mode != VX_DROP_NONE && a.in_drop_mode != VX_DROP_HASH) VX_REFUSE(r, VX_E_DTYPE, "vx_conv3d_k3: in_drop_mode %d", a.in_drop_mode);
  if (a.in_pool_flags) {
// ... 76 lines not shown
```

values_amd/csrc/convT_route.h:

```cpp
#pragma once
#include <stddef.h>
#include <stdint.h>
#include <stdio.h>

#include "../../include/values_amd.h"
#include "host_checks.h"

enum ConvTKernel { CONVT_MFMA = 0, CONVT_S16, CONVT_ROWS, CONVT_GENERIC, CONVT_NKERNELS };

#define CONVT_MFMA_INSTANCES(X) X(16, 4) X(16, 8) X(32, 4) X(32, 8) X(64, 4) X(64, 8) X(128, 4)
#define CONVT_S16_INSTANCES(X) X(64, 4) X(128, 2)
#define CONVT_ROWS_INSTANCES(X) X(16) X(32)

constexpr int convT_key(int cin, int rt = 0) { return cin * 16 + rt; }
static inline bool convT_instance_exists(int kernel, int cin, int rt, int mask) {
  if (cin < 0 || cin > 128 || rt < 0 || rt >= 16 || (mask != 0 && mask != 1)) return false;
#define CONVT_EXISTS_CASE(...) case convT_key(__VA_ARGS__):
  switch (kernel) {
    case CONVT_MFMA: switch (convT_key(cin, rt)) { CONVT_MFMA_INSTANCES(CONVT_EXISTS_CASE) return true; default: return false; }
    case CONVT_S16:  switch (convT_key(cin, rt)) { CONVT_S16_INSTANCES(CONVT_EXISTS_CASE) return true; default: return false; }
    case CONVT_ROWS: switch (convT_key(cin, rt)) { CONVT_ROWS_INSTANCES(CONVT_EXISTS_CASE) return !mask; default: return false; }
    case CONVT_GENERIC: return cin == 0 && rt == 0 && !mask;
  }
#undef CONVT_EXISTS_CASE
  return false;
}

constexpr int CT_CO = 8;
constexpr int64_t CONVT_DECODE_NVOX = 1ll << 27;
constexpr int64_t CONVT_DECODE_PRODUCT = 1ll << 32;
constexpr int CONVT_GRID_CUS = 256, CONVT_MFMA_PER_CU = 32, CONVT_S16_WGS = 512;
constexpr int CONVT_ROWS_MAX_WGS = 4096, CONVT_GENERIC_MAX_WGS = 8192;

static inline bool convT_layer_ok(int Cin, int Cout) { return Cin > 0 && Cout > 0 && Cin % 4 == 0 && Cout % CT_CO == 0; }
static inline int64_t convT_packed_floats(int Cin, int Cout) {
  if (!convT_layer_ok(Cin, Cout)) return -1;
  const vx_wide v = (vx_wide)Cin * Cout * 8;
  return v > (vx_wide)INT64_MAX ? -1 : (int64_t)v;
}

struct ConvTTiles { int kernel, rt; };
static inline bool convT_tile_rule(int Cin, int Cout, const vx_config& cfg, ConvTTiles* t) {
  const int rt48 = Cout % 16 ? 4 : 8;
  if (Cin == 16 || Cin == 32) { *t = {CONVT_MFMA, rt48}; return true; }
  if (Cin == 64) { *t = cfg.conv_fp32 == 0 ? ConvTTiles{CONVT_S16, 4} : ConvTTiles{CONVT_MFMA, rt48}; return true; }
  if (Cin == 128) { *t = cfg.conv_fp32 == 0 ? ConvTTiles{CONVT_S16, 2} : ConvTTiles{CONVT_MFMA, 4}; return true; }
  return false;
}
static inline bool convT_rows_rule(int Cin, int Cout) {
  return (Cin == 16 || Cin == 32) && Cout <= 128 && 256 % (Cout / 2) == 0;
}

struct ConvTRoute {
  int kernel;
  int cin, rt, mask;
  int grid_x, grid_y;
  int ncoltiles;
  int64_t nvox;
  int64_t total;
  unsigned mW, mH, mD;
  char err[200];
};

static inline int convT_route(const vx_convT_args& a, const vx_config& cfg, ConvTRoute* r) {
  r->err[0] = 0;
  if (!a.in || !a.w_packed || !a.bias || !a.out) VX_REFUSE(r, VX_E_NULL, "vx_convT_k2s2: null tensor");
  if (!convT_layer_ok(a.Cin, a.Cout)) VX_REFUSE(r, VX_E_SHAPE, "vx_convT_k2s2: Cin=%d (mult of 4) Cout=%d (mult of 8)", a.Cin, a.Cout);
  if (a.N <= 0 || a.D <= 0 || a.H <= 0 || a.W <= 0) VX_REFUSE(r, VX_E_SHAPE, "vx_convT_k2s2: empty tensor");
  if (a.in_pitch % 4 || a.in_pitch < a.Cin) VX_REFUSE(r, VX_E_ALIGN, "vx_convT_k2s2: input pitch");
  if (a.out_xblk) {
    if ((a.out_xblk != 1 && a.out_xblk != 2 && a.out_xblk != 4) || (2 * (int64_t)a.W) % a.out_xblk || (a.out_half != 0 && a.out_half != 1))
      VX_REFUSE(r, VX_E_SHAPE, "vx_convT_k2s2: bad concat layout (xblk=%d, half=%d)", a.out_xblk, a.out_half);
  } else if (a.out_pitch % 4 || a.out_coff % 4 || a.out_pitch < (int64_t)a.out_coff + a.Cout) {
    VX_REFUSE(r, VX_E_ALIGN, "vx_convT_k2s2: pitches/offsets must be multiples of 4 floats");
  }
  if (a.drop_mode == VX_DROP_MASK && !a.drop_mask) VX_REFUSE(r, VX_E_NULL, "vx_convT_k2s2: mask mode without mask");
  if ((vx_wide)a.D * a.H * a.W * 8 * a.Cout >= ((vx_wide)1 << 32)) VX_REFUSE(r, VX_E_SHAPE, "vx_convT_k2s2: sample too large");
  r->nvox = (int64_t)a.N * a.D * a.H * a.W;
  r->kernel = -1;
  r->cin = r->rt = r->ncoltiles = 0;
  r->mask = 0;
  r->total = 0;
  r->mW = r->mH = r->mD = 0;

  const int64_t dmax = a.W > a.H ? (a.W > a.D ? a.W : a.D) : (a.H > a.D ? a.H : a.D);
  ConvTTiles t = {-1, 0};
  if (r->nvox < CONVT_DECODE_NVOX && (vx_wide)r->nvox * dmax < CONVT_DECODE_PRODUCT && convT_tile_rule(a.Cin, a.Cout, cfg, &t)) {
    r->kernel = t.kernel; r->cin = a.Cin; r->rt = t.rt;
    r->mask = a.drop_mode == VX_DROP_MASK;
    if (!convT_instance_exists(r->kernel, r->cin, r->rt, r->mask)) VX_REFUSE(r, VX_E_SHAPE, "vx_convT_k2s2: no such instance");
    r->ncoltiles = (int)((r->nvox + 15) / 16);
    r->grid_y = (a.Cout / 2) / t.rt;
    const int wgs = t.kernel == CONVT_S16 ? CONVT_S16_WGS : CONVT_GRID_CUS * CONVT_MFMA_PER_CU;
    const int cap = (wgs + r->grid_y - 1) / r->grid_y;
    r->grid_x = (r->ncoltiles + 3) / 4;
    if (r->grid_x > cap) r->grid_x = cap;
    r->mW = vx_magic_or0(a.W); r->mH = vx_magic_or0(a.H); r->mD = vx_magic_or0(a.D);
    return VX_OK;
  }
  if ((int64_t)a.N * 2 * a.D >= (1ll << 31)) VX_REFUSE(r, VX_E_SHAPE, "vx_convT_k2s2: N * 2 D must stay below 2^31");
  if (convT_rows_rule(a.Cin, a.Cout)) {
    r->kernel = CONVT_ROWS; r->cin = a.Cin;
    if (!convT_instance_exists(r->kernel, r->cin, 0, 0)) VX_REFUSE(r, VX_E_SHAPE, "vx_convT_k2s2: no such instance");
    r->total = (int64_t)((vx_wide)r->nvox * 2 * (a.Cout / 4));
    const int64_t bx = (r->total + 255) / 256;
    r->grid_x = bx > CONVT_ROWS_MAX_WGS ? CONVT_ROWS_MAX_WGS : (int)bx;
    r->grid_y = 4;
    return VX_OK;
  }
  r->kernel = CONVT_GENERIC;
  const int64_t bx = (r->nvox + 255) / 256;
  r->grid_x = bx > CONVT_GENERIC_MAX_WGS ? CONVT_GENERIC_MAX_WGS : (int)bx;
  r->grid_y = 4 * (a.Cout / CT_CO);
  return VX_OK;
}

static inline int convT_route_name(const ConvTRoute& r, char* buf, int cap) {
  if (cap < 0) cap = 0;
  const char* m = r.mask ? "true" : "false";
  switch (r.kernel) {
    case CONVT_MFMA: return snprintf(buf, cap, "convT_k2s2_mfma_kernel<%d,%d,%s>", r.cin, r.rt, m);
    case CONVT_S16: return snprintf(buf, cap, "convT_k2s2_s16_kernel<%d,%d,%s>", r.cin, r.rt, m);
    case CONVT_ROWS: return snprintf(buf, cap, "convT_k2s2_rows_kernel");
  }
  return snprintf(buf, cap, "convT_k2s2_kernel");
}
```

values_amd/csrc/convtranspose.hip:

```cpp
#include "common.h"
#include <stdlib.h>
#include "convT_route.h"

__device__ __forceinline__ float* convT_out_ptr(const vx_convT_args& a, size_t orow, int ox, int OW, int c) {
  if (a.out_xblk) {
    const int xb = a.out_xblk;
    return a.out + orow * (2 * (size_t)OW * a.Cout) + ((ox / xb) * 2 + a.out_half) * xb * a.Cout + (ox % xb) * a.Cout + c;
  }
  return a.out + (orow * OW + ox) * a.out_pitch + a.out_coff + c;
}

__global__ __launch_bounds__(256) void convT_k2s2_kernel(vx_convT_args a, int64_t nvox_in) {
  const int ngroups = a.Cout / CT_CO;
  const int cgp = blockIdx.y % ngroups;
  const int dzy = blockIdx.y / ngroups;
  const int dz = dzy >> 1, dy = dzy & 1;
  const int co0 = cgp * CT_CO;
  const float* __restrict__ wp = a.w_packed + (size_t)dzy * a.Cin * 2 * a.Cout;
  const int OD = a.D * 2, OH = a.H * 2, OW = a.W * 2;

  for (int64_t i = blockIdx.x * (int64_t)blockDim.x + threadIdx.x; i < nvox_in; i += (int64_t)gridDim.x * blockDim.x) {
    int64_t r = i;
    const int x = r % a.W; r /= a.W;
    const int y = r % a.H; r /= a.H;
// ... 136 lines not shown
    const float* __restrict__ xin = a.in + (size_t)v * a.in_pitch + 4 * g;
#pragma unroll
    for (int q = 0; q < Q; ++q) dst[q] = *reinterpret_cast<const f32x4*>(xin + 16 * q);
  };
  constexpr bool PF = CIN <= 32;
  constexpr bool HB = PF || RT <= 4;
  f32x4 biasr[HB ? RT : 1];
  if constexpr (HB) {
#pragma unroll
    for (int rt = 0; rt < RT; ++rt) biasr[rt] = *reinterpret_cast<const f32x4*>(a.bias + oco[rt]);
  }
  f32x4 xnext[Q];
  if constexpr (PF) {
    const int ct0 = blockIdx.x * 4 + wave;
    load_x(ct0 < ncoltiles ? ct0 : ncoltiles - 1, xnext);
  }
  const uint32_t seed0 = vx_seed_of(a, a.drop_seed);
  for (int ct = blockIdx.x * 4 + wave; ct < ncoltiles; ct += wstride) {
    const int v = ct * 16 + m;
    const bool ok = v < nvox_in;
    const int vc = ok ? v : nvox_in - 1;
    f32x4 xv[Q];
    if constexpr (PF) {
#pragma unroll
      for (int q = 0; q < Q; ++q) xv[q] = xnext[q];
      const int ctn = ct + wstride;
      load_x(ctn < ncoltiles ? ctn : ncoltiles - 1, xnext);
    } else {
      load_x(ct, xv);
    }
    unsigned r = (unsigned)vc, q;
    q = vx_magic_div(r, dc.mW); const int x = (int)(r - q * (unsigned)a.W); r = q;
    q = vx_magic_div(r, dc.mH); const int y = (int)(r - q * (unsigned)a.H); r = q;
    q = vx_magic_div(r, dc.mD); const int z = (int)(r - q * (unsigned)a.D);
    const int n = (int)q;
    const vx_dkey dkey = vx_drop_key(seed0, a.drop_layer, (uint32_t)n);
#pragma unroll
    for (int rt = 0; rt < RT; ++rt) {
      f32x4 acc;
      if constexpr (HB) acc = biasr[rt];
      else acc = *reinterpret_cast<const f32x4*>(a.bias + oco[rt]);
#pragma unroll
      for (int q = 0; q < Q; ++q)
#pragma unroll
        for (int j = 0; j < 4; ++j) acc = __builtin_amdgcn_mfma_f32_16x16x4f32(wreg[rt][q][j], xv[q][j], acc, 0, 0, 0);
      const int pos = opos[rt];
      const int oz = 2 * z + (pos >> 2), oy = 2 * y + ((pos >> 1) & 1), ox = 2 * x + (pos & 1);
      const size_t orow = ((size_t)n * OD + oz) * OH + oy;
      if (a.act == VX_ACT_RELU) {
#pragma unroll
        for (int j = 0; j < 4; ++j) acc[j] = fmaxf(acc[j], 0.f);
      } else if (a.act == VX_ACT_LRELU) {
#pragma unroll
        for (int j = 0; j < 4; ++j) acc[j] = fmaxf(acc[j], 0.01f * acc[j]);
      }
      if (a.drop_mode == VX_DROP_HASH) {
        const uint32_t bits = vx_drop_bits4(dkey, (uint32_t)(((oz * OH + oy) * OW + ox) * a.Cout + oco[rt]));
#pragma unroll
        for (int j = 0; j < 4; ++j) acc[j] *= __uint_as_float((bits << (30 - j)) & 0x40000000u);
      }
      if constexpr (MASK) {
        const uint32_t mk = *reinterpret_cast<const uint32_t*>(a.drop_mask + (orow * OW + ox) * a.Cout + oco[rt]);
#pragma unroll
        for (int j = 0; j < 4; ++j) acc[j] = ((mk >> (8 * j)) & 0xFFu) ? 2.f * acc[j] : 0.f;
      }
      float* op;
      if (a.out_xblk)
        op = a.out + orow * (2 * (size_t)OW * a.Cout) +
             ((((ox >> xs) * 2 + a.out_half) << xs) + (ox & (a.out_xblk - 1))) * a.Cout + oco[rt];
      else
        op = a.out + (orow * OW + ox) * a.out_pitch + a.out_coff + oco[rt];
      *reinterpret_cast<f32x4*>(op) = acc;
      rmax = fmaxf(fmaxf(rmax, fmaxf(fabsf(acc[0]), fabsf(acc[1]))), fmaxf(fabsf(acc[2]), fabsf(acc[3])));
    }
  }
  if (a.range_flag) {
#pragma unroll
    for (int off = 32; off >= 1; off >>= 1) rmax = fmaxf(rmax, __shfl_xor(rmax, off, 64));
    if (lane == 0 && !(rmax < 32768.f)) atomicMax(a.range_flag, __float_as_uint(rmax));
  }
}

#include "s16_common.h"
template <int CIN, int RT, bool MASK = false>
__global__ __launch_bounds__(256) void convT_k2s2_s16_kernel(vx_convT_args a, int ncoltiles, int nvox_in, ConvTDecode dc) {
  constexpr int Q = CIN / 32;
  const int tid = threadIdx.x, lane = tid & 63, wave = tid >> 6;
  const int m = lane & 15, g = lane >> 4;
  const int OW = a.W * 2, OH = a.H * 2, OD = a.D * 2;
  const int rt0 = blockIdx.y * RT;
  f16x8 wh[RT][Q], wl[RT][Q];
  float rmax = 0.f;
#pragma unroll
  for (int rt = 0; rt < RT; ++rt) {
    const int row = 16 * (rt0 + rt) + m;
    const int pos = row / a.Cout, co = row % a.Cout;
    const float* wp = a.w_packed + (size_t)(pos >> 1) * CIN * 2 * a.Cout + (pos & 1) * a.Cout + co;
#pragma unroll
    for (int q = 0; q < Q; ++q)
#pragma unroll
      for (int j = 0; j < 8; ++j) {
        const float w = wp[(size_t)(32 * q + 8 * g + j) * 2 * a.Cout];
        const float c = fminf(fmaxf(w, -65504.f), 65504.f);
        if (!(fabsf(w) <= 65504.f)) rmax = __builtin_inff();
        const _Float16 h = (_Float16)c;
        wh[rt][q][j] = h;
        wl[rt][q][j] = (_Float16)((c - (float)h) * 2048.f);
      }
  }
  int opos[RT], oco[RT];
#pragma unroll
  for (int rt = 0; rt < RT; ++rt) {
    const int row = 16 * (rt0 + rt) + 4 * g;
    opos[rt] = row / a.Cout;
    oco[rt] = row % a.Cout;
  }
  const int xs = a.out_xblk ? __builtin_ctz((unsigned)a.out_xblk) : 0;
  const int wstride = (int)gridDim.x * 4;
  auto load_x = [&](int ct, f32x4* dst) {
    int v = ct * 16 + m;
    if (v >= nvox_in) v = nvox_in - 1;
    const float* __restrict__ xin = a.in + (size_t)v * a.in_pitch + 8 * g;
#pragma unroll
    for (int q = 0; q < Q; ++q) {
      dst[2 * q] = *reinterpret_cast<const f32x4*>(xin + 32 * q);
      dst[2 * q + 1] = *reinterpret_cast<const f32x4*>(xin + 32 * q + 4);
    }
  };
  f32x4 xnext[2 * Q];
  {
    const int ct0 = blockIdx.x * 4 + wave;
    load_x(ct0 < ncoltiles ? ct0 : ncoltiles - 1, xnext);
  }
  const uint32_t seed0 = vx_seed_of(a, a.drop_seed);
  const f32x4 zero = {0.f, 0.f, 0.f, 0.f};
  for (int ct = blockIdx.x * 4 + wave; ct < ncoltiles; ct += wstride) {
    const int v = ct * 16 + m;
    const int vc = v < nvox_in ? v : nvox_in - 1;
    f16x8 bh[Q], bl[Q];
#pragma unroll
    for (int q = 0; q < Q; ++q) {
      typedef unsigned u32x2 __attribute__((ext_vector_type(2)));
      f16x4 h0, l0, h1, l1;
      vx_split4(xnext[2 * q], h0, l0);
      vx_split4(xnext[2 * q + 1], h1, l1);
      const u32x2 a0 = __builtin_bit_cast(u32x2, h0), a1 = __builtin_bit_cast(u32x2, h1);
      const u32x2 c0 = __builtin_bit_cast(u32x2, l0), c1 = __builtin_bit_cast(u32x2, l1);
      bh[q] = __builtin_bit_cast(f16x8, (u32x4){a0[0], a0[1], a1[0], a1[1]});
      bl[q] = __builtin_bit_cast(f16x8, (u32x4){c0[0], c0[1], c1[0], c1[1]});
    }
    {
      const int ctn = ct + wstride;
      load_x(ctn < ncoltiles ? ctn : ncoltiles - 1, xnext);
    }
    __builtin_amdgcn_sched_barrier(0);
    asm volatile("s_nop 7" ::: "memory");
    __builtin_amdgcn_sched_barrier(0);
    unsigned r = (unsigned)vc, qq;
    qq = vx_magic_div(r, dc.mW); const int x = (int)(r - qq * (unsigned)a.W); r = qq;
    qq = vx_magic_div(r, dc.mH); const int y = (int)(r - qq * (unsigned)a.H); r = qq;
    qq = vx_magic_div(r, dc.mD); const int z = (int)(r - qq * (unsigned)a.D);
    const int n = (int)qq;
    const vx_dkey dkey = vx_drop_key(seed0, a.drop_layer, (uint32_t)n);
#pragma unroll
    for (int rt = 0; rt < RT; ++rt) {
      f32x4 acc = *reinterpret_cast<const f32x4*>(a.bias + oco[rt]);
      f32x4 accx = zero;
#pragma unroll
      for (int q = 0; q < Q; ++q) {
        acc = __builtin_amdgcn_mfma_f32_16x16x32_f16(wh[rt][q], bh[q], acc, 0, 0, 0);
        accx = __builtin_amdgcn_mfma_f32_16x16x32_f16(wh[rt][q], bl[q], accx, 0, 0, 0);
        accx = __builtin_amdgcn_mfma_f32_16x16x32_f16(wl[rt][q], bh[q], accx, 0, 0, 0);
      }
#pragma unroll
      for (int j = 0; j < 4; ++j) acc[j] = fmaf(accx[j], 1.0f / 2048.f, acc[j]);
      const int pos = opos[rt];
      const int oz = 2 * z + (pos >> 2), oy = 2 * y + ((pos >> 1) & 1), ox = 2 * x + (pos & 1);
      const size_t orow = ((size_t)n * OD + oz) * OH + oy;
      if (a.act == VX_ACT_RELU) {
#pragma unroll
        for (int j = 0; j < 4; ++j) acc[j] = fmaxf(acc[j], 0.f);
      } else if (a.act == VX_ACT_LRELU) {
#pragma unroll
        for (int j = 0; j < 4; ++j) acc[j] = fmaxf(acc[j], 0.01f * acc[j]);
      }
      if (a.drop_mode == VX_DROP_HASH) {
        const uint32_t bits = vx_drop_bits4(dkey, (uint32_t)(((oz * OH + oy) * OW + ox) * a.Cout + oco[rt]));
#pragma unroll
        for (int j = 0; j < 4; ++j) acc[j] *= __uint_as_float((bits << (30 - j)) & 0x40000000u);
      }
      if constexpr (MASK) {
        const uint32_t mk = *reinterpret_cast<const uint32_t*>(a.drop_mask + (orow * OW + ox) * a.Cout + oco[rt]);
#pragma unroll
        for (int j = 0; j < 4; ++j) acc[j] = ((mk >> (8 * j)) & 0xFFu) ? 2.f * acc[j] : 0.f;
      }
      float* op;
      if (a.out_xblk)
        op = a.out + orow * (2 * (size_t)OW * a.Cout) +
             ((((ox >> xs) * 2 + a.out_half) << xs) + (ox & (a.out_xblk - 1))) * a.Cout + oco[rt];
      else
        op = a.out + (orow * OW + ox) * a.out_pitch + a.out_coff + oco[rt];
      *reinterpret_cast<f32x4*>(op) = acc;
      rmax = fmaxf(fmaxf(rmax, fmaxf(fabsf(acc[0]), fabsf(acc[1]))), fmaxf(fabsf(acc[2]), fabsf(acc[3])));
    }
  }
  if (a.range_flag) {
#pragma unroll
    for (int off = 32; off >= 1; off >>= 1) rmax = fmaxf(rmax, __shfl_xor(rmax, off, 64));
    if (lane == 0 && !(rmax < 32768.f)) atomicMax(a.range_flag, __float_as_uint(rmax));
  }
}

static const char* convT_kname(const ConvTRoute& r) {
  char buf[128];
  convT_route_name(r, buf, (int)sizeof(buf));
  return vx_kname("%s", buf);
}

template <int FAMILY, int CIN, int RT, bool MASK>
static void launch_convT_instance(const ConvTRoute& r, const vx_convT_args& a, hipStream_t s) {
  static const char* kname = convT_kname(r);
  vx_note_kernel(kname);
  const ConvTDecode dc = {r.mW, r.mH, r.mD};
  const dim3 grid((unsigned)r.grid_x, (unsigned)r.grid_y);
  if constexpr (FAMILY == CONVT_S16)
    hipLaunchKernelGGL((convT_k2s2_s16_kernel<CIN, RT, MASK>), grid, dim3(256), 0, s, a, r.ncoltiles, (int)r.nvox, dc);
  else
    hipLaunchKernelGGL((convT_k2s2_mfma_kernel<CIN, RT, MASK>), grid, dim3(256), 0, s, a, r.ncoltiles, (int)r.nvox, dc);
}

template <int FAMILY, int CIN, int RT>
static int launch_convT_tiles(const ConvTRoute& r, const vx_convT_args& a, hipStream_t s) {
  if (r.mask) launch_convT_instance<FAMILY, CIN, RT, true>(r, a, s);
  else launch_convT_instance<FAMILY, CIN, RT, false>(r, a, s);
  VX_CHECK_LAUNCH(FAMILY == CONVT_S16 ? "vx_convT_k2s2(s16)" : "vx_convT_k2s2(mfma)");
  return VX_OK;
}

__global__ void pack_convT_kernel(const float* __restrict__ w, float* __restrict__ out, int Cin, int Cout, int64_t total) {
  for (int64_t i = blockIdx.x * (int64_t)blockDim.x + threadIdx.x; i < total; i += (int64_t)gridDim.x * blockDim.x) {
    int64_t r = i;
    const int co = r % Cout; r /= Cout;
    const int dx = r % 2; r /= 2;
    const int ci = r % Cin; r /= Cin;
    const int dy = r % 2; r /= 2;
    const int dz = (int)r;
    out[i] = w[(((size_t)ci * Cout + co) * 2 + dz) * 4 + dy * 2 + dx];
  }
}

extern "C" int64_t vx_convT_k2s2_packed_floats(int Cin, int Cout) { return convT_packed_floats(Cin, Cout); }

extern "C" int vx_pack_convT_k2s2(const float* w_torch, float* w_packed, int Cin, int Cout, vx_stream_t stream) {
  if (!w_torch || !w_packed) VX_FAIL(VX_E_NULL, "vx_pack_convT_k2s2: null pointer");
  const int64_t total = convT_packed_floats(Cin, Cout);
  if (total < 0) VX_FAIL(VX_E_SHAPE, "vx_pack_convT_k2s2: Cin=%d (mult of 4) Cout=%d (mult of 8)", Cin, Cout);
  const int64_t nb = (total - 1) / 256 + 1;
  const int blocks = nb > 4096 ? 4096 : (int)nb;
  hipLaunchKernelGGL(pack_convT_kernel, dim3(blocks), dim3(256), 0, (hipStream_t)stream, w_torch, w_packed, Cin, Cout, total);
  VX_CHECK_LAUNCH("vx_pack_convT_k2s2");
  return VX_OK;
}

static int route_or_fail(const vx_convT_args* ap, ConvTRoute* r) {
  if (!ap) VX_FAIL(VX_E_NULL, "vx_convT_k2s2: null args");
  const int rc = convT_route(*ap, vx_cfg(), r);
  if (rc != VX_OK) VX_FAIL(rc, "%s", r->err);
  return VX_OK;
}

extern "C" int vx_convT_k2s2_route(const vx_convT_args* ap, char* kernel_name, int cap, vx_convT_route_info* info) {
  ConvTRoute r;
  const int rc = route_or_fail(ap, &r);
  if (rc != VX_OK) return rc;
  if (kernel_name && cap > 0) convT_route_name(r, kernel_name, cap);
  if (info) *info = {r.grid_x, r.grid_y};
  return VX_OK;
}

extern "C" int vx_convT_k2s2(const vx_convT_args* ap, vx_stream_t stream) {
  ConvTRoute r;
  const int rc = route_or_fail(ap, &r);
  if (rc != VX_OK) return rc;
  hipStream_t s = (hipStream_t)stream;
  const dim3 grid((unsigned)r.grid_x, (unsigned)r.grid_y);
#define CONVT_LAUNCH_MFMA(CIN, RT) case convT_key(CIN, RT): return launch_convT_tiles<CONVT_MFMA, CIN, RT>(r, *ap, s);
#define CONVT_LAUNCH_S16(CIN, RT) case convT_key(CIN, RT): return launch_convT_tiles<CONVT_S16, CIN, RT>(r, *ap, s);
#define CONVT_LAUNCH_ROWS(CIN) case convT_key(CIN): hipLaunchKernelGGL(convT_k2s2_rows_kernel<CIN>, grid, dim3(256), 0, s, *ap, r.total); break;
  switch (r.kernel) {
    case CONVT_MFMA: switch (convT_key(r.cin, r.rt)) { CONVT_MFMA_INSTANCES(CONVT_LAUNCH_MFMA) } break;
    case CONVT_S16: switch (convT_key(r.cin, r.rt)) { CONVT_S16_INSTANCES(CONVT_LAUNCH_S16) } break;
    case CONVT_ROWS: {
      static const char* kname = convT_kname(r);
      vx_note_kernel(kname);
      switch (convT_key(r.cin)) { CONVT_ROWS_INSTANCES(CONVT_LAUNCH_ROWS) }
      VX_CHECK_LAUNCH("vx_convT_k2s2");
      return VX_OK;
    }
    case CONVT_GENERIC: {
      static const char* kname = convT_kname(r);
      vx_note_kernel(kname);
      hipLaunchKernelGGL(convT_k2s2_kernel, grid, dim3(256), 0, s, *ap, r.nvox);
      VX_CHECK_LAUNCH("vx_convT_k2s2");
      return VX_OK;
    }
  }
#undef CONVT_LAUNCH_MFMA
#undef CONVT_LAUNCH_S16
#undef CONVT_LAUNCH_ROWS
  VX_FAIL(VX_E_SHAPE, "vx_convT_k2s2: no such instance");
}
```

values_amd/csrc/lib.cpp:

```cpp
#include <stdarg.h>
#include <stdio.h>
#include <stdlib.h>
#include <string.h>

#include "../../include/values_amd.h"

static thread_local char g_err[512] = "";

void vx_set_error(const char* fmt, ...) {
  va_list ap;
  va_start(ap, fmt);
  vsnprintf(g_err, sizeof(g_err), fmt, ap);
  va_end(ap);
}

static thread_local const char* g_last_kernel = nullptr;
void vx_note_kernel(const char* name) { g_last_kernel = name; }
const char* vx_last_kernel() { return g_last_kernel; }
const char* vx_kname(const char* fmt, ...) {
  char buf[256];
  va_list ap;
  va_start(ap, fmt);
  vsnprintf(buf, sizeof(buf), fmt, ap);
  va_end(ap);
  char* p = (char*)malloc(strlen(buf) + 1);
  strcpy(p, buf);
  return p;
}

#include <mutex>
#include <stdlib.h>
#include <string.h>

static vx_config g_cfg;
static std::once_flag g_cfg_once;

static int env_int(const char* name, int dflt) {
  const char* e = getenv(name);
  if (!e || !*e) return dflt;
  char* end = nullptr;
  const long v = strtol(e, &end, 0);
  return end == e ? 1 : (int)v;
}

static void cfg_from_env() {
  memset(&g_cfg, 0, sizeof(g_cfg));
  g_cfg.conv_fp32 = env_int("VX_CONV_FP32", 0);
  g_cfg.s16_no_prenorm = env_int("VX_S16_NO_PRENORM", 0);
  g_cfg.s16_no_xp8 = env_int("VX_S16_NO_XP8", 0);
  g_cfg.s16_skip_raw = env_int("VX_S16_SKIP_RAW", 1);
  g_cfg.no_head_fusion = env_int("VX_NO_HEAD_FUSION", 0);
  g_cfg.s16_no_upfuse = env_int("VX_S16_NO_UPFUSE", 0);
  g_cfg.s16_no_poolfuse = env_int("VX_S16_NO_POOLFUSE", 0);
  g_cfg.storage16 = env_int("VX_STORAGE16", 0);
  g_cfg.s16_generic = env_int("VX_S16_GENERIC", 0);
  g_cfg.s16_no_zc16 = env_int("VX_S16_NO_ZC16", 0);
  g_cfg.s16_no_halves = env_int("VX_S16_NO_HALVES", 0);
  g_cfg.s16_no_deep = env_int("VX_S16_NO_DEEP", 0);
  g_cfg.s16_no_l1dma = env_int("VX_S16_NO_L1DMA", 0);
  g_cfg.c2s_no_wide = env_int("VX_C2S_NO_WIDE", 0);
  g_cfg.c2s_no_oct = env_int("VX_C2S_NO_OCT", 0);
}

const vx_config& vx_cfg() {
  std::call_once(g_cfg_once, cfg_from_env);
  return g_cfg;
}

extern "C" int vx_get_config(vx_config* out) {
  if (!out) { vx_set_error("vx_get_config: null"); return VX_E_NULL; }
  *out = vx_cfg();
  return VX_OK;
}

extern "C" int vx_set_config(const vx_config* cfg) {
  if (!cfg) { vx_set_error("vx_set_config: null"); return VX_E_NULL; }
  if (cfg->conv_fp32 < 0 || cfg->conv_fp32 > 2) { vx_set_error("vx_set_config: conv_fp32 %d", cfg->conv_fp32); return VX_E_DTYPE; }
  (void)vx_cfg();
  g_cfg = *cfg;
  return VX_OK;
}

extern "C" const char* vx_last_kernel_name(void) { return g_last_kernel ? g_last_kernel : ""; }
extern "C" int vx_version(void) { return 906;  }
extern "C" const char* vx_last_error_string(void) { return g_err; }
```

values_amd/csrc/unet3d_forward.hip:

```cpp
#include "conv3d_internal.h"

namespace {
struct Level { int D, H, W, C; int64_t nvox; };

struct Plan {
  Level lv[5];
  float *A[4], *B[4], *CAT[4], *P[5], *C0, *C1;
  float *stats, *mean, *rstd;
  float *mean0, *rstd0;
  float *meanS[4], *rstdS[4];
  size_t bytes;
};

static size_t align_up(size_t v) { return (v + 255) & ~(size_t)255; }

static void make_plan(Plan& p, int N, int D, int H, int W, int F, char* base) {
  size_t off = 0;
  auto carve = [&](size_t floats) {
    float* q = base ? (float*)(base + off) : nullptr;
    off += align_up(floats * sizeof(float));
    return q;
  };
  for (int l = 0; l < 5; ++l) {
    p.lv[l].D = D >> l; p.lv[l].H = H >> l; p.lv[l].W = W >> l; p.lv[l].C = F << l;
// ... 9 lines not shown
  for (int l = 1; l < 5; ++l) p.P[l] = carve((size_t)N * p.lv[l].nvox * p.lv[l - 1].C);
  p.C0 = carve((size_t)N * p.lv[4].nvox * p.lv[4].C);
  p.C1 = carve((size_t)N * p.lv[4].nvox * p.lv[4].C);
  size_t smax = 0;
  for (int l = 0; l < 4; ++l) {
    size_t t = (size_t)vx_conv3d_k3_tiles(p.lv[l].D, p.lv[l].H, p.lv[l].W);
    if (l == 0) {
      size_t t1 = (size_t)vx_conv3d_k3_c1_tiles(p.lv[0].D, p.lv[0].H, p.lv[0].W);
      if (t1 > t) t = t1;
    }
    const size_t e = (size_t)N * t * p.lv[l].C * 2;
    if (e > smax) smax = e;
  }
  p.stats = carve(smax);
  p.mean = carve((size_t)N * p.lv[3].C);
  p.rstd = carve((size_t)N * p.lv[3].C);
  p.mean0 = carve((size_t)N * p.lv[0].C);
  p.rstd0 = carve((size_t)N * p.lv[0].C);
  for (int l = 0; l < 4; ++l) {
    p.meanS[l] = l == 0 ? p.mean0 : carve((size_t)N * p.lv[l].C);
    p.rstdS[l] = l == 0 ? p.rstd0 : carve((size_t)N * p.lv[l].C);
  }
  p.bytes = off;
}
}

extern "C" size_t vx_unet3d_workspace_bytes(int N, int D, int H, int W, int F) {
  if (N <= 0 || D <= 0 || H <= 0 || W <= 0 || F <= 0) return 0;
  Plan p;
  make_plan(p, N, D, H, W, F, nullptr);
  return p.bytes;
}

namespace {
struct Prof {
  static constexpr int MAXL = 96;
  hipEvent_t ev[2 * MAXL];
  const char* name[MAXL];
  const char* kernel[MAXL];
  int n = 0;
  hipStream_t s;
};
thread_local Prof* g_prof = nullptr;
thread_local char g_prof_labels[Prof::MAXL][192];
}

#define VX_TRY(expr)            \
  do {                          \
    int rc_ = (expr);           \
    if (rc_ != VX_OK) return rc_; \
  } while (0)

#define VX_STEP(label, expr)                                                       \
  do {                                                                             \
    Prof* pf_ = g_prof;                                                            \
    if (pf_ && pf_->n < Prof::MAXL) { vx_note_kernel(nullptr); (void)hipEventRecord(pf_->ev[2 * pf_->n], pf_->s); }  \
    int rc_ = (expr);                                                              \
    if (rc_ != VX_OK) return rc_;                                                  \
    if (pf_ && pf_->n < Prof::MAXL) {                                              \
      (void)hipEventRecord(pf_->ev[2 * pf_->n + 1], pf_->s);                             \
      pf_->kernel[pf_->n] = vx_last_kernel();                                      \
      pf_->name[pf_->n++] = (label);                                               \
    }                                                                              \
  } while (0)

namespace {
int xblk_of(int W) { return W % 4 == 0 ? 4 : (W % 2 == 0 ? 2 : 1); }

struct Flow {
  bool inorm;
  int ich;
  int rep;
  bool shared;
  bool fuse_head;
  bool pre[4];
  bool presplit;
  bool skip_raw[4];
  bool pooled[4];
  bool poolfin1;
  bool halves[4];
  bool fuse_up;
  bool fuse_up1;
  bool split_out[4];
  bool planar1;
  bool st16;
  int products_c12, products_e11, products_e12;
};

Flow decide_flow(const vx_unet3d_weights* w, const vx_unet3d_run* r, const Plan& p) {
  const vx_config& cfg = vx_cfg();
  const int F = w->F, dm = r->drop_mode;
  const Level* lv = p.lv;
  const bool hashed = dm != VX_DROP_MASK;
  Flow f = {};
  f.inorm = !w->no_instancenorm;
  f.ich = w->in_channels > 1 ? w->in_channels : 1;
  f.rep = r->repeat > 0 ? r->repeat : 1;
  f.shared = !r->src && !r->flip && f.rep > 1 && r->N % f.rep == 0;
  f.fuse_head = w->num_classes <= 4 && vx_conv3d_k3_head_fusable(F, F) && !cfg.no_head_fusion;
  f.pre[0] = hashed && !cfg.s16_no_prenorm && F == 8 && f.inorm && vx_conv3d_k3_prologue_ok(lv[0].D, lv[0].H, lv[0].W, F, F);
  for (int l = 1; l < 4; ++l)
    f.pre[l] = f.inorm && hashed && !cfg.s16_no_prenorm && vx_conv3d_k3_prologue_ok(lv[l].D, lv[l].H, lv[l].W, lv[l].C, lv[l].C);
  f.presplit = f.shared && f.pre[0] && vx_conv3d_k3_presplit_ok(lv[0].D, lv[0].H, lv[0].W, F, F);
  f.skip_raw[0] = f.pre[0] && cfg.s16_skip_raw && vx_conv3d_k3_prologue_ok(lv[0].D, lv[0].H, lv[0].W, 2 * F, F);
  f.pooled[0] = f.skip_raw[0] && vx_conv3d_k3_poolfuse_ok(lv[0].D, lv[0].H, lv[0].W, F, F);
  f.poolfin1 = f.pooled[0] && vx_conv3d_k3_poolfin_ok(F, 2 * F);
  for (int l = 1; l < 4; ++l) {
    const Level& L = lv[l];
    f.skip_raw[l] = f.pooled[l] = f.inorm && hashed && !cfg.s16_no_prenorm && cfg.s16_skip_raw &&
                                  vx_conv3d_k3_pool_layout(L.D, L.H, L.W, L.C, L.C) == 2 &&
                                  vx_conv3d_k3_skip_prologue_ok(L.D, L.H, L.W, 2 * L.C, L.C, xblk_of(L.W));
  }
  f.halves[1] = f.skip_raw[1] && lv[1].C == 16 && w->split_w[0] && w->split_w[1] && !cfg.s16_no_halves &&
                w->split_family == vx_conv3d_k3_family(16, 16) && vx_conv3d_k3_acc_ok(lv[1].D, lv[1].H, lv[1].W, 16, 16);
  f.fuse_up = hashed && F == 8 && vx_conv3d_k3_upfuse_ok(lv[0].D, lv[0].H, lv[0].W, 2 * F, F);
  f.fuse_up1 = f.halves[1] && w->up3_zc16 && hashed && vx_conv3d_k3_upfuse_ok(lv[1].D, lv[1].H, lv[1].W, 16, 16) == 2;
  f.split_out[1] = f.fuse_up;
  f.split_out[2] = f.fuse_up1;
  f.planar1 = f.fuse_up1 && !cfg.s16_no_l1dma && vx_conv3d_k3_planar_ok(lv[1].D, lv[1].H, lv[1].W, 16, 16);
  f.st16 = cfg.storage16 && dm == VX_DROP_HASH && F == 8 && f.fuse_head && cfg.conv_fp32 == 0 &&
           vx_conv3d_k3_prologue_ok(lv[0].D, lv[0].H, lv[0].W, F, F);
  const bool one = f.st16 && cfg.storage16 == 2;
  f.products_c12 = one && f.presplit && f.pooled[0];
  f.products_e11 = one && f.skip_raw[0] && f.fuse_up && w->up_fused;
  f.products_e12 = one;
  return f;
}
}

extern "C" int vx_unet3d_forward(const vx_unet3d_weights* w, const vx_unet3d_run* r, vx_stream_t stream) {
  if (!w || !r) VX_FAIL(VX_E_NULL, "vx_unet3d_forward: null argument");
  if (!r->x || !r->logits || !r->workspace) VX_FAIL(VX_E_NULL, "vx_unet3d_forward: null tensor/workspace");
  const int N = r->N, D = r->D, H = r->H, W = r->W, F = w->F, NC = w->num_classes;
  if (N <= 0 || D <= 0 || H <= 0 || W <= 0) VX_FAIL(VX_E_SHAPE, "vx_unet3d_forward: empty batch");
  if (D % 16 || H % 16 || W % 16)
    VX_FAIL(VX_E_SHAPE, "vx_unet3d_forward: spatial size (%d,%d,%d) must be divisible by 16 (4 poolings; InstanceNorm "
            "needs > 1 voxel at the 8x level)", D, H, W);
  if (F != 8 && F != 16 && F != 32) VX_FAIL(VX_E_SHAPE, "vx_unet3d_forward: initial_filter_size %d unsupported (8,16,32)", F);
  if (NC <= 0) VX_FAIL(VX_E_SHAPE, "vx_unet3d_forward: num_classes %d", NC);
  if (r->drop_mode < 0 || r->drop_mode > 2) VX_FAIL(VX_E_DTYPE, "vx_unet3d_forward: drop_mode %d", r->drop_mode);
  if ((((uintptr_t)r->workspace) & 255u) != 0) VX_FAIL(VX_E_ALIGN, "vx_unet3d_forward: workspace must be 256-byte aligned");
  for (int i = 0; i < 18; ++i)
    if (!w->conv_w[i] || !w->conv_b[i]) VX_FAIL(VX_E_NULL, "vx_unet3d_forward: conv weight %d missing", i);
  if (w->in_channels < 0 || w->in_channels > 8) VX_FAIL(VX_E_SHAPE, "vx_unet3d_forward: in_channels %d (1 .. 8)", w->in_channels);
  for (int i = 0; i < 4; ++i)
    if (!w->up_w[i] || !w->up_b[i]) VX_FAIL(VX_E_NULL, "vx_unet3d_forward: transposed-conv weight %d missing", i);
  if (!w->final_w || !w->final_b) VX_FAIL(VX_E_NULL, "vx_unet3d_forward: final weights missing");
  if (r->drop_mode == VX_DROP_MASK)
    for (int i = 0; i < 17; ++i)
      if (!r->masks[i]) VX_FAIL(VX_E_NULL, "vx_unet3d_forward: mask %d missing", i);

  Plan p;
  make_plan(p, N, D, H, W, F, (char*)r->workspace);
  if (p.bytes > r->workspace_bytes)
    VX_FAIL(VX_E_WORKSPACE, "vx_unet3d_forward: workspace %zu B < required %zu B", r->workspace_bytes, p.bytes);
  const Flow f = decide_flow(w, r, p);

  const int dm = r->drop_mode;
  auto mask = [&](int i) { return dm == VX_DROP_MASK ? r->masks[i] : (const uint8_t*)nullptr; };
  auto conv_args = [&](int wi, const Level& L, int Cin, int Cout, float* stats) {
    vx_conv3d_args a = {};
    a.w_packed = w->conv_w[wi]; a.bias = w->conv_b[wi]; a.w_family = w->conv_family[wi];
    a.N = N; a.D = L.D; a.H = L.H; a.W = L.W; a.Cin = Cin; a.Cout = Cout;
    a.drop_seed = r->seed; a.seed_dev = r->seed_dev;
    a.stats_partial = stats; a.range_flag = stats ? nullptr : r->range_flag;
    a.out_half = 1;
    return a;
  };
  auto set_drop = [&](vx_conv3d_args& a, int act, int layer) {
    a.act = act; a.drop_mode = dm; a.drop_layer = (uint32_t)layer; a.drop_mask = mask(layer);
  };
  auto set_pre = [&](vx_conv3d_args& a, int layer, int rep, const float* mean, const float* rstd) {
    a.in_mean = mean; a.in_rstd = rstd; a.in_repeat = rep;
    a.in_drop_mode = dm; a.in_drop_seed = r->seed; a.in_drop_layer = (uint32_t)layer;
  };
  auto norm_args = [&](const float* x, int C, const Level& L, int drop_layer, bool normalise) {
    vx_norm_args a = {};
    a.x = x; a.x_pitch = C; a.x_half = 1; a.out_half = 1; a.pool_pitch = C;
    a.mean = normalise ? p.mean : nullptr; a.rstd = normalise ? p.rstd : nullptr;
    a.range_flag = normalise ? nullptr : r->range_flag;
    a.N = N; a.D = L.D; a.H = L.H; a.W = L.W; a.C = C;
    a.act = VX_ACT_LRELU;
    a.drop_mode = drop_layer >= 0 ? dm : VX_DROP_NONE; a.drop_seed = r->seed; a.drop_layer = (uint32_t)(drop_layer >= 0 ? drop_layer : 0);
    a.drop_mask = drop_layer >= 0 ? mask(drop_layer) : nullptr;
    a.seed_dev = r->seed_dev;
    return a;
  };
  auto convT = [&](const float* in, int ui, float* out, int out_pitch, const Level& Lin, int Cin, int Cout, int act,
                   int drop_layer, bool dense) {
    vx_convT_args a = {};
    a.range_flag = r->range_flag;
    a.seed_dev = r->seed_dev;
    a.out_xblk = dense ? 0 : xblk_of(2 * Lin.W); a.out_half = 0;
    a.in = in; a.in_pitch = Cin; a.w_packed = w->up_w[ui]; a.bias = w->up_b[ui];
    a.out = out; a.out_pitch = out_pitch; a.out_coff = 0;
    a.N = N; a.D = Lin.D; a.H = Lin.H; a.W = Lin.W; a.Cin = Cin; a.Cout = Cout;
    a.act = act;
    a.drop_mode = drop_layer >= 0 ? dm : VX_DROP_NONE;
    a.drop_seed = r->seed; a.drop_layer = (uint32_t)(drop_layer >= 0 ? drop_layer : 0);
    a.drop_mask = drop_layer >= 0 ? mask(drop_layer) : nullptr;
    return vx_convT_k2s2(&a, stream);
// ... 21 lines not shown
                                "finalize:contr_3_1", "finalize:contr_3_2", "finalize:contr_4_1", "finalize:contr_4_2"};
  static const char* kPoolFin[4] = {"poolfin:contr_1_2", "poolfin:contr_2_2", "poolfin:contr_3_2", "poolfin:contr_4_2"};
  static const char* kUp[4] = {"center.4", "upscale4", "upscale3", "upscale2"};
  float* const out1 = f.shared && !f.skip_raw[0] ? p.CAT[0] : p.A[0];
  const int fan = f.shared ? f.rep : 1;
  for (int l = 0; l < 4; ++l) {
    const Level& L = p.lv[l];
    const int C = L.C;
    const int ntiles = vx_conv3d_k3_tiles_for(L.D, L.H, L.W, C);
    if (l == 0) {
      const int n1 = N / fan;
      const int ntiles1 = f.ich == 1 ? vx_conv3d_k3_c1_tiles(L.D, L.H, L.W) : ntiles;
      VX_STEP(kConv[0], first_conv(out1, n1, f.shared ? 1 : f.rep, f.inorm ? p.stats : nullptr));
      if (f.inorm) VX_STEP(kFin[0], vx_instnorm_finalize(p.stats, n1, ntiles1, C, L.nvox, 1e-5f, p.mean, p.rstd, stream));
      if (f.presplit)
        VX_STEP("presplit:contr_1_1", vx_prenorm_split(out1, p.mean, p.rstd, n1, L.nvox, dm == VX_DROP_HASH ? 2.f : 1.f, stream));
      if (!f.pre[0]) {
        vx_norm_args n = norm_args(out1, C, L, 0, f.inorm);
        n.out = p.A[0]; n.out_pitch = C;
        VX_STEP(kNorm[0], vx_norm_act_drop_pool_bcast(&n, fan, stream));
      }
    } else {
      vx_conv3d_args a = conv_args(2 * l, L, C / 2, C, f.inorm ? p.stats : nullptr);
      a.in = p.P[l]; a.in_pitch = C / 2; a.out = p.A[l]; a.out_pitch = C;
      if (!f.inorm) set_drop(a, VX_ACT_LRELU, 2 * l);
      if (l == 1 && f.poolfin1) {
        a.in = p.B[0]; a.in_pool_flags = pool_flags(0);
        set_pre(a, 1, 1, p.mean0, p.rstd0);
      }
      VX_STEP(l == 1 && f.poolfin1 ? "poolfin+contr_2_1" : kConv[2 * l], vx_conv3d_k3(&a, stream));
      if (f.inorm) {
        VX_STEP(kFin[2 * l], vx_instnorm_finalize(p.stats, N, ntiles, C, L.nvox, 1e-5f, p.mean, p.rstd, stream));
        if (!f.pre[l]) {
          vx_norm_args n = norm_args(p.A[l], C, L, 2 * l, true);
          n.out = p.A[l]; n.out_pitch = C;
          VX_STEP(kNorm[2 * l], vx_norm_act_drop_pool_bcast(&n, 1, stream));
        }
      }
    }
    if (!f.inorm) {
      vx_conv3d_args a = conv_args(2 * l + 1, L, C, C, nullptr);
      a.in = p.A[l]; a.in_pitch = C; a.out = p.B[l]; a.out_pitch = C;
      set_drop(a, VX_ACT_LRELU, 2 * l + 1);
      VX_STEP(kConv[2 * l + 1], vx_conv3d_k3(&a, stream));
      vx_norm_args n = norm_args(p.B[l], C, L, -1, false);
      n.act = VX_ACT_NONE;
      n.out = p.CAT[l]; n.out_pitch = 2 * C; n.out_coff = C; n.out_xblk = xblk_of(L.W); n.pool_out = p.P[l + 1];
      VX_STEP(kNorm[2 * l + 1], vx_norm_act_drop_pool_bcast(&n, 1, stream));
      continue;
    }
    vx_conv3d_args a = conv_args(2 * l + 1, L, C, C, p.stats);
    a.in = p.A[l]; a.in_pitch = C; a.out = p.B[l]; a.out_pitch = C;
    if (f.pre[l]) {
      if (l == 0) a.in = out1;
      set_pre(a, 2 * l, l == 0 ? fan : 1, p.mean, p.rstd);
    }
    a.in_split = l == 0 && f.presplit;
    if (l == 0) a.products = f.products_c12;
    if (f.skip_raw[l]) {
      if (f.halves[l]) a.out = p.CAT[l] + (size_t)N * L.nvox * C;
      else { a.out = p.CAT[l]; a.out_xblk = xblk_of(L.W); }
    }
    if (f.pooled[l]) {
      a.pool_out = p.B[l]; a.pool_flags = pool_flags(l);
      set_drop(a, VX_ACT_NONE, 2 * l + 1);
    }
    VX_STEP(kConv[2 * l + 1], vx_conv3d_k3(&a, stream));
    if (l == 0 && f.skip_raw[0]) {
      VX_STEP(kFin[1], vx_instnorm_finalize(p.stats, N, ntiles, C, L.nvox, 1e-5f, p.mean0, p.rstd0, stream));
      if (!f.pooled[0]) {
        vx_norm_args n = norm_args(p.CAT[0], C, L, 1, true);
        n.mean = p.mean0; n.rstd = p.rstd0; n.x_xblk = xblk_of(L.W); n.pool_out = p.P[1];
        VX_STEP("pool:contr_1_2", vx_norm_act_drop_pool_bcast(&n, 1, stream));
      } else if (!f.poolfin1) {
        VX_STEP(kPoolFin[0], vx_pool_finish(p.B[0], pool_flags(0), p.mean0, p.rstd0, p.P[1], C, N, p.lv[1].nvox, dm == VX_DROP_HASH, stream));
      }
    } else if (f.skip_raw[l]) {
      const vx_stat_src st = {p.stats, ntiles, 1e-5f, (int64_t)L.nvox, p.meanS[l], p.rstdS[l]};
      VX_STEP(kPoolFin[l], vx_pool_finish_z_stats(p.B[l], pool_flags(l), &st, p.P[l + 1], C, N, L.D / 2, (int64_t)(L.H / 2) * (L.W / 2),
                                                  dm == VX_DROP_HASH, stream));
    } else {
      vx_norm_args n = norm_args(p.B[l], C, L, 2 * l + 1, true);
      n.out = p.CAT[l]; n.out_pitch = 2 * C; n.out_coff = C; n.out_xblk = xblk_of(L.W); n.pool_out = p.P[l + 1];
      if (C <= 512) {
        n.mean = nullptr; n.rstd = nullptr;
        const vx_stat_src st = {p.stats, ntiles, 1e-5f, (int64_t)L.nvox, p.mean, p.rstd};
        VX_STEP(kNorm[2 * l + 1], vx_norm_act_drop_pool_stats(&n, &st, stream));
      } else {
        VX_STEP(kFin[2 * l + 1], vx_instnorm_finalize(p.stats, N, ntiles, C, L.nvox, 1e-5f, p.mean, p.rstd, stream));
        VX_STEP(kNorm[2 * l + 1], vx_norm_act_drop_pool_bcast(&n, 1, stream));
      }
    }
  }
  {
    const Level& L4 = p.lv[4];
    const int C3 = p.lv[3].C, C4 = L4.C;
    vx_conv3d_args a = conv_args(8, L4, C3, C4, nullptr);
    a.in = p.P[4]; a.in_pitch = C3; a.out = p.C0; a.out_pitch = C4; a.act = VX_ACT_RELU;
    VX_STEP(kConv[8], vx_conv3d_k3(&a, stream));
    vx_conv3d_args b = conv_args(9, L4, C4, C4, nullptr);
    b.in = p.C0; b.in_pitch = C4; b.out = p.C1; b.out_pitch = C4; b.act = VX_ACT_RELU;
    VX_STEP(kConv[9], vx_conv3d_k3(&b, stream));
    VX_STEP(kUp[0], convT(p.C1, 0, p.CAT[3], 2 * C3, L4, C4, C3, VX_ACT_RELU, 8, false));
  }
  for (int l = 3; l >= 0; --l) {
    const Level& L = p.lv[l];
    const int C = L.C;
    const int wi = 10 + 2 * (3 - l);
    const int dl = 9 + 2 * (3 - l);
    if (f.halves[l]) {
      vx_conv3d_args a = conv_args(wi, L, C, C, nullptr);
      a.w_packed = w->split_w[1]; a.w_family = w->split_family;
      a.in = p.CAT[l] + (size_t)N * L.nvox * C; a.in_pitch = C; a.out = p.A[l]; a.out_pitch = C;
      set_pre(a, 2 * l + 1, 1, p.meanS[l], p.rstdS[l]);
      a.range_flag = nullptr;
      VX_STEP("expand_2_1(skip half)", vx_conv3d_k3(&a, stream));
      vx_conv3d_args b = conv_args(wi, L, C, C, nullptr);
      b.w_packed = w->split_w[0]; b.w_family = w->split_family;
      b.in = p.CAT[l]; b.in_pitch = C; b.out = p.A[l]; b.out_pitch = C; b.acc_in = p.A[l]; b.acc_pitch = C;
      set_drop(b, VX_ACT_LRELU, dl);
      if (f.fuse_up1) {
        b.in = p.B[l + 1]; b.up_in = p.B[l + 1]; b.up_pitch = 2 * C; b.up_w = w->up3_zc16; b.up_b = w->up_b[2];
        b.up_split = 1;
        b.up_fused = w->up3_fused;
      }
      if (f.planar1) { b.out = p.CAT[l]; b.out_planar = 1; }
      VX_STEP(f.fuse_up1 ? "upscale3+expand_2_1(up half)" : "expand_2_1(up half)", vx_conv3d_k3(&b, stream));
    } else {
      vx_conv3d_args a = conv_args(wi, L, 2 * C, C, nullptr);
      a.in = p.CAT[l]; a.in_pitch = 2 * C; a.in_xblk = xblk_of(L.W); a.out = p.A[l]; a.out_pitch = C;
      set_drop(a, VX_ACT_LRELU, dl);
      if (f.skip_raw[l]) set_pre(a, 2 * l + 1, 1, p.meanS[l], p.rstdS[l]);
      if (l == 0 && f.fuse_up) {
        a.up_in = p.B[1]; a.up_w = w->up_w[3]; a.up_b = w->up_b[3]; a.up_pitch = 2 * C;
        a.up_fused = w->up_fused;
        a.up_split = 1;
      }
      if (l == 0) { a.out_f16 = f.st16; a.products = f.products_e11; }
      VX_STEP(l == 0 && f.fuse_up ? "upscale2+expand_1_1" : kConv[wi], vx_conv3d_k3(&a, stream));
    }
    vx_conv3d_args a = conv_args(wi + 1, L, C, C, nullptr);
    a.in = p.A[l]; a.in_pitch = C; a.out = p.B[l]; a.out_pitch = C;
    set_drop(a, VX_ACT_LRELU, dl + 1);
    if (l == 1 && f.planar1) { a.in = p.CAT[l]; a.in_planar = 1; }
    a.out_split = f.split_out[l];
    if (l == 0) { a.in_f16 = f.st16; a.products = f.products_e12; }
    if (l == 0 && f.fuse_head) {
      a.out = nullptr;
      a.head_out = r->logits; a.head_w = w->final_w; a.head_b = w->final_b; a.head_C = NC; a.head_dst = r->dst; a.head_flip = r->flip;
    }
    VX_STEP(l == 0 && f.fuse_head ? "expand_1_2+final" : kConv[wi + 1], vx_conv3d_k3(&a, stream));
    if (l > 0 && !(l == 1 && f.fuse_up) && !(l == 2 && f.fuse_up1))
      VX_STEP(kUp[4 - l], convT(p.B[l], 4 - l, p.CAT[l - 1], f.halves[l - 1] ? C / 2 : C, L, C, C / 2, VX_ACT_NONE, -1, f.halves[l - 1]));
  }
  if (!f.fuse_head)
    VX_STEP("final", vx_conv1x1_ncdhw(p.B[0], F, w->final_w, w->final_b, r->logits, N, D, H, W, F, NC, r->dst, r->flip, stream));
  return VX_OK;
}

extern "C" int vx_unet3d_forward_profiled(const vx_unet3d_weights* w, const vx_unet3d_run* r, vx_stream_t stream,
                                          int max_launches, float* ms, const char** labels, int* n_launches) {
  if (!ms || !labels || !n_launches) VX_FAIL(VX_E_NULL, "vx_unet3d_forward_profiled: null output");
  Prof pf;
  pf.s = (hipStream_t)stream;
  for (int i = 0; i < 2 * Prof::MAXL; ++i) {
    hipError_t e = hipEventCreate(&pf.ev[i]);
    if (e != hipSuccess) VX_FAIL((int)e, "hipEventCreate: %s", hipGetErrorString(e));
  }
  g_prof = &pf;
  int rc = vx_unet3d_forward(w, r, stream);
  g_prof = nullptr;
  if (rc == VX_OK) {
    hipError_t e = hipStreamSynchronize(pf.s);
    if (e != hipSuccess) { vx_set_error("hipStreamSynchronize: %s", hipGetErrorString(e)); rc = (int)e; }
  }
  int n = 0;
  if (rc == VX_OK) {
    for (; n < pf.n && n < max_launches; ++n) {
      float t = 0.f;
      (void)hipEventElapsedTime(&t, pf.ev[2 * n], pf.ev[2 * n + 1]);
      ms[n] = t;
      snprintf(g_prof_labels[n], sizeof(g_prof_labels[n]), "%s|%s", pf.name[n], pf.kernel[n] ? pf.kernel[n] : "?");
      labels[n] = g_prof_labels[n];
    }
  }
  *n_launches = n;
  for (int i = 0; i < 2 * Prof::MAXL; ++i) (void)hipEventDestroy(pf.ev[i]);
  return rc;
}
```

values_amd/unet3d.py:

```python
from __future__ import annotations

import ctypes as C
from typing import List, Optional, Sequence

import torch
import torch.nn as nn

from . import _lib

CONV_ORDER = ["contr_1_1.0", "contr_1_2.0", "contr_2_1.0", "contr_2_2.0", "contr_3_1.0", "contr_3_2.0",
              "contr_4_1.0", "contr_4_2.0", "center.0", "center.2", "expand_4_1.0", "expand_4_2.0",
              "expand_3_1.0", "expand_3_2.0", "expand_2_1.0", "expand_2_2.0", "expand_1_1.0", "expand_1_2.0"]
UP_ORDER = ["center.4", "upscale4", "upscale3", "upscale2"]
DROPOUT_ORDER = ["contr_1_1", "contr_1_2", "contr_2_1", "contr_2_2", "contr_3_1", "contr_3_2", "contr_4_1",
                 "contr_4_2", "center", "expand_4_1", "expand_4_2", "expand_3_1", "expand_3_2", "expand_2_1",
                 "expand_2_2", "expand_1_1", "expand_1_2"]


def _block(cin, cout, k, norm, p):
    layers = [nn.Conv3d(cin, cout, k, padding=1)]
    if norm:
        layers.append(nn.InstanceNorm3d(cout))
    layers += [nn.LeakyReLU(inplace=True), nn.Dropout(p=p)]
    return nn.Sequential(*layers)


class UNet3D(nn.Module):
    def __init__(self, num_classes: int, in_channels: int = 1, initial_filter_size: int = 8, kernel_size: int = 3,
                 do_instancenorm: bool = True, do_dropout: bool = False, aleatoric_loss: bool = False):
        super().__init__()
        if kernel_size != 3:
            raise NotImplementedError("values_amd.UNet3D: only kernel_size=3 (every shipped config) has a HIP kernel")
        if not 1 <= in_channels <= 8:
            raise NotImplementedError("values_amd.UNet3D: in_channels must be 1 .. 8")
        if initial_filter_size not in (8, 16, 32):
            raise NotImplementedError("values_amd.UNet3D: initial_filter_size must be 8, 16 or 32")
        self.num_classes = num_classes
        self.aleatoric_loss = aleatoric_loss
        self.in_channels = in_channels
        self.do_instancenorm = bool(do_instancenorm)
        self.initial_filter_size = initial_filter_size
        self.dropout_prob = 0.5 if do_dropout else 0.0
        f, p = initial_filter_size, self.dropout_prob
        chans = [f, 2 * f, 4 * f, 8 * f]
        prev = in_channels
        for lvl, c in enumerate(chans, start=1):
            setattr(self, f"contr_{lvl}_1", _block(prev, c, 3, do_instancenorm, p))
            setattr(self, f"contr_{lvl}_2", _block(c, c, 3, do_instancenorm, p))
            prev = c
        center = [nn.Conv3d(8 * f, 16 * f, 3, padding=1), nn.ReLU(inplace=True),
                  nn.Conv3d(16 * f, 16 * f, 3, padding=1), nn.ReLU(inplace=True),
                  nn.ConvTranspose3d(16 * f, 8 * f, 2, stride=2), nn.ReLU(inplace=True)]
        if do_dropout:
            center.append(nn.Dropout(p=p))
        self.center = nn.Sequential(*center)
        for lvl in (4, 3, 2, 1):
            c = chans[lvl - 1]
            setattr(self, f"expand_{lvl}_1", _block(2 * c, c, 3, False, p))
            setattr(self, f"expand_{lvl}_2", _block(c, c, 3, False, p))
            if lvl > 1:
                setattr(self, f"upscale{lvl}", nn.ConvTranspose3d(c, c // 2, kernel_size=2, stride=2))
        self.final = nn.Conv3d(f, num_classes, kernel_size=1)
        if aleatoric_loss:
            self.final_aleatoric = nn.Conv3d(f, num_classes * 2, kernel_size=1)
        self.output_reconstruction_map = nn.Conv3d(f, out_channels=1, kernel_size=1)
        self._packed = None
        self._packed_key = None
        self._packed_by_mode = {}
        self._range = {}
        self._ws = {}
        self._calls = 0
        self.seed = 123

    def _param_key(self):
        return tuple((p.data_ptr(), p._version, p.dtype, str(p.device)) for p in self.parameters()) + (_lib.pack_mode(),)

    def _ensure_packed(self, device):
        key = self._param_key()
        mode = (key[-1], str(device))
        hit = self._packed_by_mode.get(mode)
        if hit is not None and hit[0] == key:
            self._packed, self._packed_key = hit[1], key
            return self._packed
        lib = _lib.load()
        sd = {k: v.detach().to(device=device, dtype=torch.float32).contiguous() for k, v in self.state_dict().items()}
        keep = []
        w = _lib.UNet3DWeights()
        st = _lib.stream_ptr()
        for i, name in enumerate(CONV_ORDER):
            wt, b = sd[name + ".weight"], sd[name + ".bias"]
            cout, cin = wt.shape[0], wt.shape[1]
            if i == 0 and cin > 1:
                wt8 = torch.zeros((cout, 8) + tuple(wt.shape[2:]), dtype=torch.float32, device=device)
                wt8[:, :cin] = wt
                wt, cin = wt8.contiguous(), 8
                n = lib.vx_conv3d_k3_packed_floats(cin, cout)
                packed = torch.empty(n, dtype=torch.float32, device=device)
                _lib.check(lib.vx_pack_conv3d_k3(_lib.ptr(wt), _lib.ptr(packed), cin, cout, st), "vx_pack_conv3d_k3")
            elif i == 0:
                packed = wt
            else:
                n = lib.vx_conv3d_k3_packed_floats(cin, cout)
                if n < 0:
                    raise _lib.VxError(f"conv {name}: Cin={cin} Cout={cout} unsupported")
                packed = torch.empty(n, dtype=torch.float32, device=device)
                _lib.check(lib.vx_pack_conv3d_k3(_lib.ptr(wt), _lib.ptr(packed), cin, cout, st), "vx_pack_conv3d_k3")
            keep += [packed, b, wt]
            w.conv_w[i] = packed.data_ptr()
            w.conv_b[i] = b.data_ptr()
            w.conv_family[i] = 0 if (i == 0 and cin == 1) else lib.vx_conv3d_k3_family(cin, cout)
        for i, name in enumerate(UP_ORDER):
            wt, b = sd[name + ".weight"], sd[name + ".bias"]
            cin, cout = wt.shape[0], wt.shape[1]
            n = lib.vx_convT_k2s2_packed_floats(cin, cout)
            packed = torch.empty(n, dtype=torch.float32, device=device)
            _lib.check(lib.vx_pack_convT_k2s2(_lib.ptr(wt), _lib.ptr(packed), cin, cout, st), "vx_pack_convT_k2s2")
            keep += [packed, b, wt]
            w.up_w[i] = packed.data_ptr()
            w.up_b[i] = b.data_ptr()
        if self.initial_filter_size == 8 and _lib.get_config().conv_fp32 == 0:
            uf = torch.empty(lib.vx_conv3d_upfused_packed_floats(), dtype=torch.float32, device=device)
            _lib.check(lib.vx_pack_conv3d_upfused(_lib.ptr(sd["expand_1_1.0.weight"]), _lib.ptr(sd["expand_1_1.0.bias"]),
                                                  _lib.ptr(sd["upscale2.weight"]), _lib.ptr(sd["upscale2.bias"]), _lib.ptr(uf), st),
                       "vx_pack_conv3d_upfused")
            keep.append(uf)
            w.up_fused = uf.data_ptr()
            w2 = sd["expand_2_1.0.weight"]
            for hidx in range(2):
                part = w2[:, 16 * hidx:16 * (hidx + 1)].contiguous()
                pk = torch.empty(lib.vx_conv3d_k3_packed_floats(16, 16), dtype=torch.float32, device=device)
                _lib.check(lib.vx_pack_conv3d_k3(_lib.ptr(part), _lib.ptr(pk), 16, 16, st), "vx_pack_conv3d_k3 (expand_2_1 half)")
                keep += [part, pk]
                w.split_w[hidx] = pk.data_ptr()
            w.split_family = lib.vx_conv3d_k3_family(16, 16)
            u3 = torch.empty(lib.vx_convT_zc16_packed_floats(), dtype=torch.float32, device=device)
            _lib.check(lib.vx_pack_convT_zc16(_lib.ptr(sd["upscale3.weight"]), _lib.ptr(u3), st), "vx_pack_convT_zc16")
            keep.append(u3)
            w.up3_zc16 = u3.data_ptr()
            if hasattr(lib, "vx_pack_conv3d_upfused_zc16"):
                u3f = torch.empty(lib.vx_conv3d_upfused_zc16_packed_floats(), dtype=torch.float32, device=device)
                _lib.check(lib.vx_pack_conv3d_upfused_zc16(_lib.ptr(w2), _lib.ptr(sd["upscale3.weight"]), _lib.ptr(sd["upscale3.bias"]),
                                                           _lib.ptr(u3f), st), "vx_pack_conv3d_upfused_zc16")
                keep.append(u3f)
                w.up3_fused = u3f.data_ptr()
        fw, fb = self._head_params(sd)
        keep += [fw, fb]
        w.final_w = fw.data_ptr()
        w.final_b = fb.data_ptr()
        w.F = self.initial_filter_size
        w.num_classes = fw.shape[0]
        w.in_channels = self.in_channels
        w.no_instancenorm = 0 if self.do_instancenorm else 1
        self._packed = (w, keep)
        self._packed_key = key
        self._packed_by_mode[mode] = (key, self._packed)
        return self._packed

    def _head_params(self, sd):
        head = "final_aleatoric" if self.aleatoric_loss else "final"
        return sd[head + ".weight"].reshape(sd[head + ".weight"].shape[0], -1).contiguous(), sd[head + ".bias"]

    def _workspace(self, N, D, H, W, device):
        geo = (N, D, H, W, str(device))
        sid = torch.cuda.current_stream(device).cuda_stream
        ent = self._ws.get(sid)
        if ent is None or ent[0] != geo:
            nbytes = _lib.load().vx_unet3d_workspace_bytes(N, D, H, W, self.initial_filter_size)
            self._ws.pop(sid, None)
            ent = (geo, torch.empty(nbytes + 256, dtype=torch.uint8, device=device))
            self._ws[sid] = ent
        ws = ent[1]
        off = (-ws.data_ptr()) % 256
        return ws, off, ws.numel() - 256

    FP16_MAX = 65504.0

    def range_max(self, reset: bool = False) -> float:
        worst = 0.0
        for flag in self._range.values():
            worst = max(worst, float(flag.view(torch.float32).item()))
            if reset:
                flag.zero_()
        return worst

    def range_reset(self):
        for flag in self._range.values():
            flag.zero_()

    def next_seed(self) -> int:
        seed = (self.seed * 1000003 + self._calls) & 0xFFFFFFFF
        self._calls += 1
        return seed

    def check_range(self, reset: bool = True):
        m = self.range_max(reset=reset)
        if not m < self.FP16_MAX:
            raise _lib.VxError(f"values_amd.UNet3D: an activation of magnitude {m:.4g} reached a split-fp16 convolution "
                               f"(limit {self.FP16_MAX}); re-run under _lib.config(conv_fp32=1)")

    def dropout_layer_shapes(self, D, H, W):
        f = self.initial_filter_size
        enc = [(f << l, (D >> l, H >> l, W >> l)) for l in range(4) for _ in range(2)]
        dec = [(f << l, (D >> l, H >> l, W >> l)) for l in (3, 2, 1, 0) for _ in range(2)]
        return enc + [(8 * f, (D >> 3, H >> 3, W >> 3))] + dec

    def hash_dropout_masks(self, seed: int, N: int, D: int, H: int, W: int, device=None):
        _lib.require_gpu()
        lib = _lib.load()
        dev = torch.device("cuda", torch.cuda.current_device()) if device is None else torch.device(device)
        out = []
        for layer, (c, (d, h, w)) in enumerate(self.dropout_layer_shapes(D, H, W)):
            m = torch.empty((N, d, h, w, c), dtype=torch.uint8, device=dev)
            _lib.check(lib.vx_drop_hash_mask(int(seed) & 0xFFFFFFFF, layer, N, d * h * w * c, _lib.ptr(m),
                                             _lib.stream_ptr()), "vx_drop_hash_mask")
            out.append(m.permute(0, 4, 1, 2, 3).bool())
        return out

    def forward(self, x: torch.Tensor, enable_concat: bool = True, last_layer: bool = True, *,
                n_samples: int = 1, src: Optional[torch.Tensor] = None, flip: Optional[torch.Tensor] = None,
                dst: Optional[torch.Tensor] = None, out: Optional[torch.Tensor] = None,
                dropout_masks: Optional[Sequence[torch.Tensor]] = None, seed: Optional[int] = None,
                seed_dev: Optional[torch.Tensor] = None):
        if not enable_concat or not last_layer:
            raise NotImplementedError("values_amd.UNet3D: autoencoder / feature modes are training-only and not on the HIP path")
        res = self._run(x, n_samples=n_samples, src=src, flip=flip, dst=dst, out=out, dropout_masks=dropout_masks, seed=seed,
                        seed_dev=seed_dev)
        if self.aleatoric_loss:
# ... 63 lines not shown
```

Measured before the change: 3998 volumes/s.

## Compose upscale4 transposed conv with expand_3_1 up-half into one kernel

Precomposes the 2x2x2 stride-2 transposed convolution (upscale4) with the up-channel half of the following 3x3x3 conv (expand_3_1) into effective per-parity 2x2x2 weights plus a boundary-dependent bias table. A new MFMA kernel applies these directly to the 8^3x64 decoder input and writes dense partial sums, so the upsampled 32-channel tensor is never materialised. The skip half is then run as a separate 32->32 deep conv that accumulates onto those partial sums through a new acc_in path. This removes the concat write and the read of the upsampled intermediate, at the cost of an extra partial-sum buffer round trip and split-fp16 precision in the composed weights.

```diff
diff --git a/include/values_amd.h b/include/values_amd.h
--- a/include/values_amd.h
+++ b/include/values_amd.h
@@ -213,8 +213,14 @@
   int32_t out_xblk, out_half;
   uint32_t* range_flag;
   const uint32_t* seed_dev;
+  const float* compose;
+  int32_t in_split;
 } vx_convT_args;
 int vx_convT_k2s2(const vx_convT_args* a, vx_stream_t stream);
+int64_t vx_convT_compose32_packed_floats(void);
+int vx_pack_convT_compose32(const float* w1_torch, const float* b1, const float* up_w_torch, const float* up_b, float* packed,
+                            vx_stream_t stream);
+int vx_convT_k2s2_compose_ok(int D, int H, int W, int Cin, int Cout);
 typedef struct vx_convT_route_info {
   int32_t grid_x, grid_y;
 } vx_convT_route_info;
@@ -240,6 +246,9 @@
   int32_t split_family;
   const float* up3_zc16;
   const float* up3_fused;
+  const float* up4_fused;
+  const float* split3_w;
+  int32_t split3_family;
 } vx_unet3d_weights;
 
 typedef struct vx_unet3d_run {
diff --git a/values_amd/_lib.py b/values_amd/_lib.py
--- a/values_amd/_lib.py
+++ b/values_amd/_lib.py
@@ -56,7 +56,8 @@
                 ("out", _p), ("out_pitch", _i32), ("out_coff", _i32),
                 ("N", _i32), ("D", _i32), ("H", _i32), ("W", _i32), ("Cin", _i32), ("Cout", _i32),
                 ("act", _i32), ("drop_mode", _i32), ("drop_seed", _u32), ("drop_layer", _u32), ("drop_mask", _p),
-                ("out_xblk", _i32), ("out_half", _i32), ("range_flag", _p), ("seed_dev", _p)]
+                ("out_xblk", _i32), ("out_half", _i32), ("range_flag", _p), ("seed_dev", _p),
+                ("compose", _p), ("in_split", _i32)]
 
 
 class ConvTRouteInfo(C.Structure):
@@ -124,7 +125,8 @@
 class UNet3DWeights(C.Structure):
     _fields_ = [("conv_w", _p * 18), ("conv_b", _p * 18), ("up_w", _p * 4), ("up_b", _p * 4),
                 ("final_w", _p), ("final_b", _p), ("F", _i32), ("num_classes", _i32), ("conv_family", _i32 * 18),
-                ("in_channels", _i32), ("no_instancenorm", _i32), ("up_fused", _p), ("split_w", _p * 2), ("split_family", _i32), ("up3_zc16", _p), ("up3_fused", _p)]
+                ("in_channels", _i32), ("no_instancenorm", _i32), ("up_fused", _p), ("split_w", _p * 2), ("split_family", _i32), ("up3_zc16", _p), ("up3_fused", _p),
+                ("up4_fused", _p), ("split3_w", _p), ("split3_family", _i32)]
 
 
 class UNet3DRun(C.Structure):
@@ -353,6 +355,9 @@
     "vx_pool_finish_z_stats": (_i, [_p, _p, C.POINTER(StatSrc), _p, _i, _i, _i, _i64, _i, _p]),
     "vx_convT_k2s2": (_i, [C.POINTER(ConvTArgs), _p]),
     "vx_convT_k2s2_route": (_i, [C.POINTER(ConvTArgs), C.c_char_p, _i, C.POINTER(ConvTRouteInfo)]),
+    "vx_convT_compose32_packed_floats": (_i64, []),
+    "vx_pack_convT_compose32": (_i, [_p, _p, _p, _p, _p, _p]),
+    "vx_convT_k2s2_compose_ok": (_i, [_i, _i, _i, _i, _i]),
     "vx_conv1x1_ncdhw": (_i, [_p, _i, _p, _p, _p, _i, _i, _i, _i, _i, _i, _p, _p, _p]),
     "vx_unet3d_workspace_bytes": (C.c_size_t, [_i, _i, _i, _i, _i]),
     "vx_unet3d_forward": (_i, [C.POINTER(UNet3DWeights), C.POINTER(UNet3DRun), _p]),
diff --git a/values_amd/csrc/conv3d_deep.hip b/values_amd/csrc/conv3d_deep.hip
--- a/values_amd/csrc/conv3d_deep.hip
+++ b/values_amd/csrc/conv3d_deep.hip
@@ -346,6 +346,12 @@
       const unsigned osoff = (vox0 * (unsigned)out_voxf + (unsigned)(cg * 32)) * 4u;
       const __amdgpu_buffer_rsrc_t osrd = __builtin_amdgcn_make_buffer_rsrc(
           (void*)(reinterpret_cast<char*>(kp->a.out) + (size_t)n0 * out_sample * 4), 0, VX_NUMREC, 0x00020000);
+      const bool have_acc = !STATS && kp->a.acc_in != nullptr;
+      const unsigned acc_voxf = (unsigned)kp->a.acc_pitch;
+      const unsigned acc_sample = (unsigned)(a.D * a.H * a.W) * acc_voxf;
+      const __amdgpu_buffer_rsrc_t asrd = __builtin_amdgcn_make_buffer_rsrc(
+          (void*)(const_cast<float*>(kp->a.acc_in) + (size_t)n0 * acc_sample), 0, VX_NUMREC, 0x00020000);
+      const unsigned asoff = (vox0 * acc_voxf + (unsigned)(cg * 32)) * 4u;
       float ssum[NT][4], ssq[NT][4];
       if (STATS) {
 #pragma unroll
@@ -355,6 +361,23 @@
       }
       int m_ = m;
       asm volatile("" : "+v"(m_));
+      f32x4 part[R][NT];
+      if constexpr (!STATS) {
+        if (have_acc) {
+#pragma unroll
+          for (int r = 0; r < R; ++r) {
+            int cx_, ly, lz, smp;
+            vox_of((wave * R + r) * 16 + m_, cx_, ly, lz, smp);
+            unsigned avoff_r = ((unsigned)smp * acc_sample + (unsigned)((lz * a.H + ly) * a.W + cx_) * acc_voxf + 4u * g) * 4u;
+            if constexpr (R == 2) {
+              if (n0 + smp >= a.N) avoff_r = VX_OOB;
+            }
+#pragma unroll
+            for (int nt = 0; nt < NT; ++nt)
+              part[r][nt] = __builtin_bit_cast(f32x4, __builtin_amdgcn_raw_buffer_load_b128(asrd, (int)avoff_r, (int)(asoff + (unsigned)(nt * 64)), 0));
+          }
+        }
+      }
 #pragma unroll
       for (int r = 0; r < R; ++r) {
         int cx_, ly, lz, smp;
@@ -374,6 +397,12 @@
           f32x4 v;
 #pragma unroll
           for (int j = 0; j < 4; ++j) v[j] = fmaf(accx[r][nt][j], 1.0f / 2048.f, acc[r][nt][j]);
+          if constexpr (!STATS) {
+            if (have_acc) {
+#pragma unroll
+              for (int j = 0; j < 4; ++j) v[j] += part[r][nt][j];
+            }
+          }
           if (STATS) {
 #pragma unroll
             for (int j = 0; j < 4; ++j) { ssum[nt][j] += v[j]; ssq[nt][j] = fmaf(v[j], v[j], ssq[nt][j]); }
@@ -475,7 +504,7 @@
         const f32x4 zero = {0.f, 0.f, 0.f, 0.f};
 #pragma unroll
         for (int nt = 0; nt < NT; ++nt) {
-          const f32x4 b4 = *reinterpret_cast<const f32x4*>(s_bias + cg * 32 + nt * 16 + 4 * g);
+          const f32x4 b4 = !STATS && a.acc_in ? zero : *reinterpret_cast<const f32x4*>(s_bias + cg * 32 + nt * 16 + 4 * g);
 #pragma unroll
           for (int r = 0; r < R; ++r) { acc[r][nt] = b4; accx[r][nt] = zero; }
         }
diff --git a/values_amd/csrc/conv3d_k3.hip b/values_amd/csrc/conv3d_k3.hip
--- a/values_amd/csrc/conv3d_k3.hip
+++ b/values_amd/csrc/conv3d_k3.hip
@@ -53,7 +53,10 @@
 extern "C" int vx_conv3d_k3_skip_prologue_ok(int D, int H, int W, int Cin, int Cout, int xblk) {
   return conv3d_skip_prologue_ok(D, H, W, Cin, Cout, xblk, vx_cfg());
 }
-extern "C" int vx_conv3d_k3_acc_ok(int D, int H, int W, int Cin, int Cout) { return conv3d_zc16_16to16(D, H, W, Cin, Cout, vx_cfg()) ? 1 : 0; }
+extern "C" int vx_conv3d_k3_acc_ok(int D, int H, int W, int Cin, int Cout) {
+  const vx_config& cfg = vx_cfg();
+  return (conv3d_zc16_16to16(D, H, W, Cin, Cout, cfg) || (conv_config(Cin, Cout, cfg).S16 && conv3d_deep_applies(D, H, W, Cin, Cout, cfg))) ? 1 : 0;
+}
 extern "C" int vx_conv3d_k3_planar_ok(int D, int H, int W, int Cin, int Cout) { return conv3d_zc16_16to16(D, H, W, Cin, Cout, vx_cfg()) ? 1 : 0; }
 extern "C" int vx_conv3d_k3_upfuse_ok(int D, int H, int W, int Cin, int Cout) { return conv3d_upfuse_ok(D, H, W, Cin, Cout, vx_cfg()); }
 extern "C" int vx_conv3d_k3_pool_layout(int D, int H, int W, int Cin, int Cout) { return conv3d_pool_layout(D, H, W, Cin, Cout, vx_cfg()); }
diff --git a/values_amd/csrc/conv3d_route.h b/values_amd/csrc/conv3d_route.h
--- a/values_amd/csrc/conv3d_route.h
+++ b/values_amd/csrc/conv3d_route.h
@@ -412,7 +412,7 @@
 
 static inline int route_deep(const vx_conv3d_args& a, int stat_tiles, Conv3dRoute* r) {
   if (a.head_out || a.in_split || a.in_f16 || a.out_f16 || (a.in_repeat > 1) || a.out_xblk || a.up_in || a.pool_out ||
-      a.in_pool_flags || a.acc_in)
+      a.in_pool_flags)
     return ROUTE_DECLINED;
   if (a.drop_mode == VX_DROP_MASK || !a.out) return ROUTE_DECLINED;
   DeepGeo g;
@@ -451,6 +451,12 @@
   else if (a.drop_mode == VX_DROP_HASH) { if (a.act != VX_ACT_LRELU) return ROUTE_DECLINED; epi = 1; }
   else epi = 3;
   if (a.out_split && a.stats_partial) VX_REFUSE(r, VX_E_SHAPE, "vx_conv3d_k3(deep): out_split goes with the activation epilogues");
+  if (a.acc_in) {
+    if (a.stats_partial) VX_REFUSE(r, VX_E_SHAPE, "vx_conv3d_k3(deep): partial sums (acc_in) go with the activation epilogues, not with statistics");
+    if (!vx_aligned16(a.acc_in) || a.acc_pitch % 4) VX_REFUSE(r, VX_E_ALIGN, "vx_conv3d_k3(deep): acc_in must be 16-byte aligned, its pitch a multiple of 4 floats");
+    if (a.acc_pitch < a.Cout || (vx_wide)g.ts * a.D * a.H * a.W * a.acc_pitch * 4 >= CONV3D_2GIB)
+      VX_REFUSE(r, VX_E_SHAPE, "vx_conv3d_k3(deep): acc_in pitch %d must cover the %d channels, one tile's samples stay below 2 GiB", a.acc_pitch, a.Cout);
+  }
   route_instance(r, CONV3D_DEEP, 3, R, epi, a.in_mean ? 1 : 0);
   return conv3d_instance_exists(CONV3D_DEEP, r->p, 3) ? VX_OK : ROUTE_DECLINED;
 }
diff --git a/values_amd/csrc/convT_route.h b/values_amd/csrc/convT_route.h
--- a/values_amd/csrc/convT_route.h
+++ b/values_amd/csrc/convT_route.h
@@ -5,6 +5,7 @@
 
 #include "../../include/values_amd.h"
 #include "host_checks.h"
+#include "upcompose32.h"
 
 enum ConvTKernel { CONVT_MFMA = 0, CONVT_S16, CONVT_ROWS, CONVT_GENERIC, CONVT_NKERNELS };
 
@@ -59,8 +60,18 @@
   int64_t nvox;
   int64_t total;
   unsigned mW, mH, mD;
+  int composed;
+  int lds_bytes;
   char err[200];
 };
+
+constexpr int CONVT_C32_POS = 3 * 9 * 9;
+constexpr int CONVT_C32_WIN = 2 * CONVT_C32_POS * 128;
+constexpr int CONVT_C32_LDS = CONVT_C32_WIN + 256 * 16 * 4;
+constexpr int CONVT_C32_MAX_LANES = CONVT_S16_WGS / 8;
+static inline bool convT_compose_ok(int D, int H, int W, int Cin, int Cout, const vx_config& cfg) {
+  return cfg.conv_fp32 == 0 && vx_upc32_shape_ok(D, H, W, Cin, Cout) != 0;
+}
 
 static inline int convT_route(const vx_convT_args& a, const vx_config& cfg, ConvTRoute* r) {
   r->err[0] = 0;
@@ -82,6 +93,27 @@
   r->mask = 0;
   r->total = 0;
   r->mW = r->mH = r->mD = 0;
+  r->composed = r->lds_bytes = 0;
+  if (a.in_split && !a.compose) VX_REFUSE(r, VX_E_SHAPE, "vx_convT_k2s2: in_split goes with the composed launch (compose)");
+  if (a.compose) {
+    if (!convT_compose_ok(a.D, a.H, a.W, a.Cin, a.Cout, cfg))
+      VX_REFUSE(r, VX_E_SHAPE, "vx_convT_k2s2: the composed launch is taken where vx_convT_k2s2_compose_ok (8x8x8, 64 -> 32, split-fp16 "
+                 "family); got %dx%dx%d, %d -> %d", a.D, a.H, a.W, a.Cin, a.Cout);
+    if (a.out_xblk || a.act != VX_ACT_NONE || a.drop_mode != VX_DROP_NONE)
+      VX_REFUSE(r, VX_E_SHAPE, "vx_convT_k2s2: the composed launch writes dense partial sums: no concat layout, activation or dropout");
+    if (!vx_aligned16(a.compose) || !vx_aligned16(a.in) || !vx_aligned16(a.out))
+      VX_REFUSE(r, VX_E_ALIGN, "vx_convT_k2s2: compose / in / out must be 16-byte aligned");
+    if (a.in_pitch != VX_UPC32_CC) VX_REFUSE(r, VX_E_ALIGN, "vx_convT_k2s2: the composed launch reads a dense input (pitch 64), got %d", a.in_pitch);
+    if (a.N > (1 << 24)) VX_REFUSE(r, VX_E_SHAPE, "vx_convT_k2s2: composed launch, N = %d", a.N);
+    if ((vx_wide)a.N * 4096 * a.out_pitch >= ((vx_wide)1 << 40) ) VX_REFUSE(r, VX_E_SHAPE, "vx_convT_k2s2: composed launch, output too large");
+    r->kernel = CONVT_S16; r->cin = 64; r->rt = 4; r->mask = 0;
+    r->composed = 1;
+    r->lds_bytes = CONVT_C32_LDS;
+    const int items = 4 * a.N;
+    r->grid_x = 8 * (items < CONVT_C32_MAX_LANES ? items : CONVT_C32_MAX_LANES);
+    r->grid_y = 1;
+    return VX_OK;
+  }
 
   const int64_t dmax = a.W > a.H ? (a.W > a.D ? a.W : a.D) : (a.H > a.D ? a.H : a.D);
   ConvTTiles t = {-1, 0};
diff --git a/values_amd/csrc/convtranspose.hip b/values_amd/csrc/convtranspose.hip
--- a/values_amd/csrc/convtranspose.hip
+++ b/values_amd/csrc/convtranspose.hip
@@ -242,8 +242,157 @@
 }
 
 #include "s16_common.h"
+
+__device__ __forceinline__ void convT_compose32_body(const vx_convT_args& a) {
+  extern __shared__ __attribute__((aligned(16))) unsigned char c32_lds[];
+  constexpr int PREC_B = CONVT_C32_POS * 128;
+  const int tid = threadIdx.x, lane = tid & 63;
+  const int wave = __builtin_amdgcn_readfirstlane(tid >> 6);
+  const int m = lane & 15, g = lane >> 4;
+  const int b = blockIdx.x, L = (int)gridDim.x >> 3;
+  int cls, item0;
+  if ((L & 7) == 0) { cls = (b >> 3) & 7; item0 = (b & 7) + 8 * (b >> 6); }
+  else { cls = b & 7; item0 = b >> 3; }
+  const int pz = cls >> 2, py = (cls >> 1) & 1, px = cls & 1;
+  const int rt = wave & 1, zl = wave >> 1;
+  const int items = 4 * a.N;
+
+  f16x8 wh[16], wl[16];
+  {
+    const u32x4* wp = reinterpret_cast<const u32x4*>(a.compose) + (size_t)((cls * 2 + rt) * 32) * 64 + lane;
+#pragma unroll
+    for (int ks = 0; ks < 16; ++ks) {
+      wh[ks] = __builtin_bit_cast(f16x8, wp[(2 * ks) * 64]);
+      wl[ks] = __builtin_bit_cast(f16x8, wp[(2 * ks + 1) * 64]);
+    }
+  }
+  const float* __restrict__ btab = a.compose + VX_UPC32_WHALVES / 2;
+
+  const int c4 = tid & 15;
+  u32x4* s_pw = reinterpret_cast<u32x4*>(c32_lds + CONVT_C32_WIN) + tid;
+#pragma unroll
+  for (int k4 = 0; k4 < 4; ++k4) {
+    u32x4 pw;
+#pragma unroll
+    for (int kk = 0; kk < 4; ++kk) {
+    const int k = 4 * k4 + kk;
+    const int pos = (tid >> 4) + 16 * k;
+    const int wz = pos / 81, wy = (pos / 9) % 9, wx = pos % 9;
+    const int cy = py - 1 + wy, cx = px - 1 + wx;
+    const bool ok = cy >= 0 && cy < 8 && cx >= 0 && cx < 8;
+    const unsigned ld = (unsigned)(pos * 128 + (((c4 >> 1) ^ (pos & 7)) * 16) + (c4 & 1) * 8);
+    const unsigned go = ok ? (unsigned)(((wz * 64 + cy * 8 + cx) * 64 + c4 * 4) * 4) : 0u;
+    pw[kk] = (ld >> 3) | ((go >> 4) << 12) | ((unsigned)wz << 24) | (ok ? 1u << 26 : 0u);
+    }
+    s_pw[k4 * 256] = pw;
+  }
+  const bool last_piece = (tid >> 4) + 240 < CONVT_C32_POS;
+  const bool presplit = a.in_split != 0;
+
+  int pb[4];
+#pragma unroll
+  for (int t = 0; t < 4; ++t) pb[t] = (zl * 9 + 2 * t + (m >> 3)) * 9 + (m & 7);
+  const int co = 16 * rt + 4 * g;
+  const int fx = 2 * (m & 7) + px;
+  const int bcx = fx == 0 ? 0 : (fx == 15 ? 2 : 1);
+
+  for (int it = item0; it < items; it += L) {
+    const int n = it >> 2, zq = it & 3;
+    {
+      const __amdgpu_buffer_rsrc_t srd = __builtin_amdgcn_make_buffer_rsrc(
+          (void*)(a.in + (size_t)n * (512 * 64)), 0, 512 * 64 * 4, 0x00020000);
+      const int z0 = 2 * zq + pz - 1;
+      auto request = [&](int k) {
+        const unsigned w = s_pw[(k >> 2) * 256][k & 3];
+        const int cz = z0 + (int)((w >> 24) & 3u);
+        const bool ok = (w & (1u << 26)) && cz >= 0 && cz < 8;
+        const unsigned vo = ok ? (unsigned)(z0 * 16384) + (((w >> 12) & 0xFFFu) << 4) : VX_OOB;
+        return __builtin_amdgcn_raw_buffer_load_b128(srd, (int)vo, 0, 0);
+      };
+      auto commit = [&](int k, const u32x4 v) {
+        typedef unsigned u32x2 __attribute__((ext_vector_type(2)));
+        u32x2 h2, l2;
+        if (presplit) {
+          h2 = (u32x2){v[0], v[1]};
+          l2 = (u32x2){v[2], v[3]};
+        } else {
+          f16x4 hi, lo;
+          vx_split4_s(__builtin_bit_cast(f32x4, v), hi, lo);
+          h2 = __builtin_bit_cast(u32x2, hi);
+          l2 = __builtin_bit_cast(u32x2, lo);
+        }
+        unsigned char* dst = c32_lds + ((s_pw[(k >> 2) * 256][k & 3] & 0xFFFu) << 3);
+        if (k < 15 || last_piece) {
+          *reinterpret_cast<u32x2*>(dst) = h2;
+          *reinterpret_cast<u32x2*>(dst + PREC_B) = l2;
+        }
+      };
+      u32x4 v[12];
+#pragma unroll
+      for (int k = 0; k < 12; ++k) v[k] = request(k);
+      __syncthreads();
+#pragma unroll
+      for (int k = 0; k < 4; ++k) commit(k, v[k]);
+      __builtin_amdgcn_sched_barrier(0);
+#pragma unroll
+      for (int k = 0; k < 4; ++k) v[k] = request(12 + k);
+      __builtin_amdgcn_sched_barrier(0);
+#pragma unroll
+      for (int k = 4; k < 12; ++k) commit(k, v[k]);
+#pragma unroll
+      for (int k = 0; k < 4; ++k) commit(12 + k, v[k]);
+    }
+    __syncthreads();
+    const int fz = 2 * (2 * zq + zl) + pz;
+    const int bcz = fz == 0 ? 0 : (fz == 15 ? 2 : 1);
+    f32x4 acc[4], accx[4];
+#pragma unroll
+    for (int t = 0; t < 4; ++t) {
+      const int fy = 2 * (2 * t + (m >> 3)) + py;
+      const int bcy = fy == 0 ? 0 : (fy == 15 ? 2 : 1);
+      acc[t] = *reinterpret_cast<const f32x4*>(btab + ((bcz * 3 + bcy) * 3 + bcx) * 32 + co);
+      accx[t] = (f32x4){0.f, 0.f, 0.f, 0.f};
+    }
+#pragma unroll
+    for (int tap = 0; tap < 8; ++tap) {
+      const int off = (tap >> 2) * 81 + ((tap >> 1) & 1) * 9 + (tap & 1);
+#pragma unroll
+      for (int t = 0; t < 4; ++t) {
+        const int pos = pb[t] + off;
+        const int ad = (pos << 7) | (((pos & 7) ^ g) << 4);
+#pragma unroll
+        for (int q = 0; q < 2; ++q) {
+          const unsigned char* src = c32_lds + (ad ^ (q << 6));
+          const f16x8 bh = *reinterpret_cast<const f16x8*>(src);
+          const f16x8 bl = *reinterpret_cast<const f16x8*>(src + PREC_B);
+          const int ks = 2 * tap + q;
+          acc[t] = __builtin_amdgcn_mfma_f32_16x16x32_f16(wh[ks], bh, acc[t], 0, 0, 0);
+          accx[t] = __builtin_amdgcn_mfma_f32_16x16x32_f16(wh[ks], bl, accx[t], 0, 0, 0);
+          accx[t] = __builtin_amdgcn_mfma_f32_16x16x32_f16(wl[ks], bh, accx[t], 0, 0, 0);
+        }
+      }
+      __builtin_amdgcn_sched_barrier(0);
+    }
+#pragma unroll
+    for (int t = 0; t < 4; ++t) {
+      f32x4 v;
+#pragma unroll
+      for (int j = 0; j < 4; ++j) v[j] = fmaf(accx[t][j], 1.0f / 2048.f, acc[t][j]);
+      const int fy = 2 * (2 * t + (m >> 3)) + py;
+      const size_t ovox = (((size_t)n * 16 + fz) * 16 + fy) * 16 + fx;
+      *reinterpret_cast<f32x4*>(a.out + ovox * a.out_pitch + a.out_coff + co) = v;
+    }
+  }
+}
+
 template <int CIN, int RT, bool MASK = false>
-__global__ __launch_bounds__(256) void convT_k2s2_s16_kernel(vx_convT_args a, int ncoltiles, int nvox_in, ConvTDecode dc) {
+__global__ __launch_bounds__(256) __attribute__((amdgpu_waves_per_eu(2))) void convT_k2s2_s16_kernel(vx_convT_args a, int ncoltiles, int nvox_in, ConvTDecode dc) {
+  if constexpr (CIN == 64 && RT == 4 && !MASK) {
+    if (a.compose) {
+      convT_compose32_body(a);
+      return;
+    }
+  }
   constexpr int Q = CIN / 32;
   const int tid = threadIdx.x, lane = tid & 63, wave = tid >> 6;
   const int m = lane & 15, g = lane >> 4;
@@ -383,8 +532,18 @@
   vx_note_kernel(kname);
   const ConvTDecode dc = {r.mW, r.mH, r.mD};
   const dim3 grid((unsigned)r.grid_x, (unsigned)r.grid_y);
+  if constexpr (FAMILY == CONVT_S16) {
+    if (r.lds_bytes) {
+      static bool attr = false;
+      if (!attr) {
+        (void)hipFuncSetAttribute(reinterpret_cast<const void*>(convT_k2s2_s16_kernel<CIN, RT, MASK>),
+                                  hipFuncAttributeMaxDynamicSharedMemorySize, r.lds_bytes);
+        attr = true;
+      }
+    }
+  }
   if constexpr (FAMILY == CONVT_S16)
-    hipLaunchKernelGGL((convT_k2s2_s16_kernel<CIN, RT, MASK>), grid, dim3(256), 0, s, a, r.ncoltiles, (int)r.nvox, dc);
+    hipLaunchKernelGGL((convT_k2s2_s16_kernel<CIN, RT, MASK>), grid, dim3(256), (size_t)r.lds_bytes, s, a, r.ncoltiles, (int)r.nvox, dc);
   else
     hipLaunchKernelGGL((convT_k2s2_mfma_kernel<CIN, RT, MASK>), grid, dim3(256), 0, s, a, r.ncoltiles, (int)r.nvox, dc);
 }
@@ -419,6 +578,36 @@
   const int blocks = nb > 4096 ? 4096 : (int)nb;
   hipLaunchKernelGGL(pack_convT_kernel, dim3(blocks), dim3(256), 0, (hipStream_t)stream, w_torch, w_packed, Cin, Cout, total);
   VX_CHECK_LAUNCH("vx_pack_convT_k2s2");
+  return VX_OK;
+}
+
+__global__ void pack_convT_compose32_kernel(const float* __restrict__ w1, const float* __restrict__ b1, const float* __restrict__ uw,
+                                            const float* __restrict__ ub, float* __restrict__ packed) {
+  _Float16* wh = reinterpret_cast<_Float16*>(packed);
+  float* btab = packed + VX_UPC32_WHALVES / 2;
+  const int total = VX_UPC32_WHALVES + 27 * VX_UPC32_CO;
+  for (int i = blockIdx.x * blockDim.x + threadIdx.x; i < total; i += gridDim.x * blockDim.x) {
+    if (i < VX_UPC32_WHALVES) {
+      int cls, tap, ci, co, lo;
+      vx_upc32_coords(i, &cls, &tap, &ci, &co, &lo);
+      _Float16 h, l;
+      vx_upc32_split<_Float16>(vx_upc32_weff(w1, 2 * VX_UPC32_CU, uw, VX_UPC32_CU, cls, tap, ci, co), &h, &l);
+      wh[i] = lo ? l : h;
+    } else {
+      const int e = i - VX_UPC32_WHALVES, co = e % VX_UPC32_CO, bc = e / VX_UPC32_CO;
+      btab[e] = (float)vx_upc32_btab(w1, 2 * VX_UPC32_CU, b1, ub, VX_UPC32_CU, bc / 9, (bc / 3) % 3, bc % 3, co);
+    }
+  }
+}
+
+extern "C" int64_t vx_convT_compose32_packed_floats(void) { return VX_UPC32_FLOATS; }
+extern "C" int vx_convT_k2s2_compose_ok(int D, int H, int W, int Cin, int Cout) { return convT_compose_ok(D, H, W, Cin, Cout, vx_cfg()) ? 1 : 0; }
+extern "C" int vx_pack_convT_compose32(const float* w1_torch, const float* b1, const float* up_w_torch, const float* up_b, float* packed,
+                                       vx_stream_t stream) {
+  if (!w1_torch || !b1 || !up_w_torch || !up_b || !packed) VX_FAIL(VX_E_NULL, "vx_pack_convT_compose32: null pointer");
+  if (!vx_aligned16(packed)) VX_FAIL(VX_E_ALIGN, "vx_pack_convT_compose32: packed must be 16-byte aligned");
+  hipLaunchKernelGGL(pack_convT_compose32_kernel, dim3(1028), dim3(256), 0, (hipStream_t)stream, w1_torch, b1, up_w_torch, up_b, packed);
+  VX_CHECK_LAUNCH("vx_pack_convT_compose32");
   return VX_OK;
 }
 
diff --git a/values_amd/csrc/lib.cpp b/values_amd/csrc/lib.cpp
--- a/values_amd/csrc/lib.cpp
+++ b/values_amd/csrc/lib.cpp
@@ -82,5 +82,5 @@
 }
 
 extern "C" const char* vx_last_kernel_name(void) { return g_last_kernel ? g_last_kernel : ""; }
-extern "C" int vx_version(void) { return 906;  }
+extern "C" int vx_version(void) { return 907;  }
 extern "C" const char* vx_last_error_string(void) { return g_err; }
diff --git a/values_amd/csrc/unet3d_forward.hip b/values_amd/csrc/unet3d_forward.hip
--- a/values_amd/csrc/unet3d_forward.hip
+++ b/values_amd/csrc/unet3d_forward.hip
@@ -115,6 +115,7 @@
   bool fuse_up;
   bool fuse_up1;
   bool split_out[4];
+  bool upcomp2;
   bool planar1;
   bool st16;
   int products_c12, products_e11, products_e12;
@@ -148,8 +149,14 @@
                 w->split_family == vx_conv3d_k3_family(16, 16) && vx_conv3d_k3_acc_ok(lv[1].D, lv[1].H, lv[1].W, 16, 16);
   f.fuse_up = hashed && F == 8 && vx_conv3d_k3_upfuse_ok(lv[0].D, lv[0].H, lv[0].W, 2 * F, F);
   f.fuse_up1 = f.halves[1] && w->up3_zc16 && hashed && vx_conv3d_k3_upfuse_ok(lv[1].D, lv[1].H, lv[1].W, 16, 16) == 2;
+  f.upcomp2 = w->up4_fused && w->split3_w && hashed && f.inorm && !f.skip_raw[2] && !cfg.s16_no_upfuse && !cfg.s16_no_deep &&
+              cfg.conv_fp32 == 0 && w->split3_family == vx_conv3d_k3_family(lv[2].C, lv[2].C) &&
+              vx_convT_k2s2_compose_ok(lv[3].D, lv[3].H, lv[3].W, lv[3].C, lv[2].C) &&
+              vx_conv3d_k3_acc_ok(lv[2].D, lv[2].H, lv[2].W, lv[2].C, lv[2].C) &&
+              vx_conv3d_k3_acc_ok(lv[2].D, lv[2].H, lv[2].W, 2 * lv[2].C, lv[2].C);
   f.split_out[1] = f.fuse_up;
   f.split_out[2] = f.fuse_up1;
+  f.split_out[3] = f.upcomp2;
   f.planar1 = f.fuse_up1 && !cfg.s16_no_l1dma && vx_conv3d_k3_planar_ok(lv[1].D, lv[1].H, lv[1].W, 16, 16);
   f.st16 = cfg.storage16 && dm == VX_DROP_HASH && F == 8 && f.fuse_head && cfg.conv_fp32 == 0 &&
            vx_conv3d_k3_prologue_ok(lv[0].D, lv[0].H, lv[0].W, F, F);
@@ -337,6 +344,7 @@
     } else {
       vx_norm_args n = norm_args(p.B[l], C, L, 2 * l + 1, true);
       n.out = p.CAT[l]; n.out_pitch = 2 * C; n.out_coff = C; n.out_xblk = xblk_of(L.W); n.pool_out = p.P[l + 1];
+      if (l == 2 && f.upcomp2) { n.out = p.CAT[l] + (size_t)N * L.nvox * C; n.out_pitch = C; n.out_coff = 0; n.out_xblk = 0; }
       if (C <= 512) {
         n.mean = nullptr; n.rstd = nullptr;
         const vx_stat_src st = {p.stats, ntiles, 1e-5f, (int64_t)L.nvox, p.mean, p.rstd};
@@ -381,6 +389,12 @@
       }
       if (f.planar1) { b.out = p.CAT[l]; b.out_planar = 1; }
       VX_STEP(f.fuse_up1 ? "upscale3+expand_2_1(up half)" : "expand_2_1(up half)", vx_conv3d_k3(&b, stream));
+    } else if (l == 2 && f.upcomp2) {
+      vx_conv3d_args a = conv_args(wi, L, C, C, nullptr);
+      a.w_packed = w->split3_w; a.w_family = w->split3_family;
+      a.in = p.CAT[l] + (size_t)N * L.nvox * C; a.in_pitch = C; a.out = p.A[l]; a.out_pitch = C; a.acc_in = p.A[l]; a.acc_pitch = C;
+      set_drop(a, VX_ACT_LRELU, dl);
+      VX_STEP(kConv[wi], vx_conv3d_k3(&a, stream));
     } else {
       vx_conv3d_args a = conv_args(wi, L, 2 * C, C, nullptr);
       a.in = p.CAT[l]; a.in_pitch = 2 * C; a.in_xblk = xblk_of(L.W); a.out = p.A[l]; a.out_pitch = C;
@@ -405,7 +419,13 @@
       a.head_out = r->logits; a.head_w = w->final_w; a.head_b = w->final_b; a.head_C = NC; a.head_dst = r->dst; a.head_flip = r->flip;
     }
     VX_STEP(l == 0 && f.fuse_head ? "expand_1_2+final" : kConv[wi + 1], vx_conv3d_k3(&a, stream));
-    if (l > 0 && !(l == 1 && f.fuse_up) && !(l == 2 && f.fuse_up1))
+    if (l == 3 && f.upcomp2) {
+      vx_convT_args t = {};
+      t.in = p.B[3]; t.in_pitch = C; t.in_split = 1; t.w_packed = w->up_w[1]; t.bias = w->up_b[1]; t.compose = w->up4_fused;
+      t.out = p.A[2]; t.out_pitch = C / 2;
+      t.N = N; t.D = L.D; t.H = L.H; t.W = L.W; t.Cin = C; t.Cout = C / 2;
+      VX_STEP(kUp[1], vx_convT_k2s2(&t, stream));
+    } else if (l > 0 && !(l == 1 && f.fuse_up) && !(l == 2 && f.fuse_up1))
       VX_STEP(kUp[4 - l], convT(p.B[l], 4 - l, p.CAT[l - 1], f.halves[l - 1] ? C / 2 : C, L, C, C / 2, VX_ACT_NONE, -1, f.halves[l - 1]));
   }
   if (!f.fuse_head)
diff --git a/values_amd/csrc/upcompose32.h b/values_amd/csrc/upcompose32.h
--- /dev/null
+++ b/values_amd/csrc/upcompose32.h
@@ -0,0 +1,79 @@
+#pragma once
+#include <stdint.h>
+
+#if defined(__HIPCC__) || defined(__CUDACC__)
+#define VX_UPC32_FN __host__ __device__ inline
+#else
+#define VX_UPC32_FN inline
+#endif
+
+VX_UPC32_FN void vx_upc32_tap(int p, int k, int* a, int* d) {
+  const int t = p + k - 1;
+  const int o = t < 0 ? -1 : t >> 1;
+  *d = t - 2 * o;
+  *a = o - (p - 1);
+}
+
+VX_UPC32_FN double vx_upc32_weff(const float* w1, int w1_cin, const float* uw, int CU, int cls, int tap, int ci, int co) {
+  const int pz = cls >> 2, py = (cls >> 1) & 1, px = cls & 1;
+  const int ta = tap >> 2, tb = (tap >> 1) & 1, tc = tap & 1;
+  double acc = 0.0;
+  for (int kz = 0; kz < 3; ++kz) {
+    int a, dz; vx_upc32_tap(pz, kz, &a, &dz);
+    if (a != ta) continue;
+    for (int ky = 0; ky < 3; ++ky) {
+      int b, dy; vx_upc32_tap(py, ky, &b, &dy);
+      if (b != tb) continue;
+      for (int kx = 0; kx < 3; ++kx) {
+        int c, dx; vx_upc32_tap(px, kx, &c, &dx);
+        if (c != tc) continue;
+        for (int cu = 0; cu < CU; ++cu)
+          acc += (double)w1[((size_t)co * w1_cin + cu) * 27 + kz * 9 + ky * 3 + kx] * (double)uw[((size_t)ci * CU + cu) * 8 + dz * 4 + dy * 2 + dx];
+      }
+    }
+  }
+  return acc;
+}
+
+VX_UPC32_FN double vx_upc32_btab(const float* w1, int w1_cin, const float* b1, const float* ub, int CU, int cz, int cy, int cx, int co) {
+  double acc = (double)b1[co];
+  for (int kz = 0; kz < 3; ++kz) {
+    if ((cz == 0 && kz == 0) || (cz == 2 && kz == 2)) continue;
+    for (int ky = 0; ky < 3; ++ky) {
+      if ((cy == 0 && ky == 0) || (cy == 2 && ky == 2)) continue;
+      for (int kx = 0; kx < 3; ++kx) {
+        if ((cx == 0 && kx == 0) || (cx == 2 && kx == 2)) continue;
+        for (int cu = 0; cu < CU; ++cu) acc += (double)w1[((size_t)co * w1_cin + cu) * 27 + kz * 9 + ky * 3 + kx] * (double)ub[cu];
+      }
+    }
+  }
+  return acc;
+}
+
+template <typename H>
+VX_UPC32_FN void vx_upc32_split(double x, H* hi, H* lo) {
+  const float xf = (float)x;
+  const float c = xf > 65504.f ? 65504.f : (xf < -65504.f ? -65504.f : xf);
+  const H h = (H)c;
+  *hi = h;
+  *lo = (H)((c - (float)h) * 2048.f);
+}
+
+#define VX_UPC32_CC 64
+#define VX_UPC32_CU 32
+#define VX_UPC32_CO 32
+#define VX_UPC32_WHALVES (8 * 2 * 16 * 2 * 64 * 8)
+#define VX_UPC32_FLOATS (VX_UPC32_WHALVES / 2 + 27 * VX_UPC32_CO)
+VX_UPC32_FN void vx_upc32_coords(int i, int* cls, int* tap, int* ci, int* co, int* lo) {
+  const int j = i & 7, lane = (i >> 3) & 63;
+  *lo = (i >> 9) & 1;
+  const int ks = (i >> 10) & 15, rt = (i >> 14) & 1;
+  *cls = i >> 15;
+  *tap = ks >> 1;
+  *ci = 32 * (ks & 1) + 8 * (lane >> 4) + j;
+  *co = 16 * rt + (lane & 15);
+}
+
+static inline int vx_upc32_shape_ok(int D, int H, int W, int Cin, int Cout) {
+  return D == 8 && H == 8 && W == 8 && Cin == VX_UPC32_CC && Cout == VX_UPC32_CU;
+}
diff --git a/values_amd/unet3d.py b/values_amd/unet3d.py
--- a/values_amd/unet3d.py
+++ b/values_amd/unet3d.py
@@ -66,6 +66,7 @@
         self.output_reconstruction_map = nn.Conv3d(f, out_channels=1, kernel_size=1)
         self._packed = None
         self._packed_key = None
+        self.compose_up4 = True
         self._packed_by_mode = {}
         self._range = {}
         self._ws = {}
@@ -73,11 +74,11 @@
         self.seed = 123
 
     def _param_key(self):
-        return tuple((p.data_ptr(), p._version, p.dtype, str(p.device)) for p in self.parameters()) + (_lib.pack_mode(),)
+        return tuple((p.data_ptr(), p._version, p.dtype, str(p.device)) for p in self.parameters()) + (bool(self.compose_up4), _lib.pack_mode())
 
     def _ensure_packed(self, device):
         key = self._param_key()
-        mode = (key[-1], str(device))
+        mode = (key[-1], key[-2], str(device))
         hit = self._packed_by_mode.get(mode)
         if hit is not None and hit[0] == key:
             self._packed, self._packed_key = hit[1], key
@@ -143,6 +144,18 @@
                                                            _lib.ptr(u3f), st), "vx_pack_conv3d_upfused_zc16")
                 keep.append(u3f)
                 w.up3_fused = u3f.data_ptr()
+            if self.compose_up4 and hasattr(lib, "vx_pack_convT_compose32"):
+                w3 = sd["expand_3_1.0.weight"]
+                u4f = torch.empty(lib.vx_convT_compose32_packed_floats(), dtype=torch.float32, device=device)
+                _lib.check(lib.vx_pack_convT_compose32(_lib.ptr(w3), _lib.ptr(sd["expand_3_1.0.bias"]), _lib.ptr(sd["upscale4.weight"]),
+                                                       _lib.ptr(sd["upscale4.bias"]), _lib.ptr(u4f), st), "vx_pack_convT_compose32")
+                part = w3[:, 32:64].contiguous()
+                pk = torch.empty(lib.vx_conv3d_k3_packed_floats(32, 32), dtype=torch.float32, device=device)
+                _lib.check(lib.vx_pack_conv3d_k3(_lib.ptr(part), _lib.ptr(pk), 32, 32, st), "vx_pack_conv3d_k3 (expand_3_1 skip half)")
+                keep += [u4f, part, pk]
+                w.up4_fused = u4f.data_ptr()
+                w.split3_w = pk.data_ptr()
+                w.split3_family = lib.vx_conv3d_k3_family(32, 32)
         fw, fb = self._head_params(sd)
         keep += [fw, fb]
         w.final_w = fw.data_ptr()
```

Result: no change. 4010 volumes/s (median of 6 runs) (+0.3%).
